# SeanSoraghan/Feature-Extractor

Hardware: AMD Instinct MI355X
Metric: frames/sec (1024-pt FFT, 10-feature bundle) (higher is better)
Workload: dtype f32

## Files before the change

### feature-extractor_amd/build.py

```python
import os
import shutil
import subprocess

HERE = os.path.dirname(os.path.abspath(__file__))
CSRC = os.path.join(HERE, "csrc")
LIB_DIR = os.path.join(HERE, "lib")
LIB_PATH = os.path.join(LIB_DIR, "libfx_hip.so")
HOST_SOURCES = ["fx_capi.cpp", "fx_plan.cpp", "fx_stream.cpp", "fx_comm.cpp", "fx_osc_sender.cpp"]
SOURCES = ["fx_kernels.hip", "fx_offline.hip", "fx_reblock.hip", "fx_osc.hip", "fx_taps.hip", "fx_interleave.hip", "fx_events.hip", "fx_tracks.hip", "fx_osc_table.hip", "fx_osc_bundle.hip"] + HOST_SOURCES
UNITS = [("fx_kernels.hip", "fx_kernels_small.o", ["-DFX_PART=1", "-mllvm", "-amdgpu-use-amdgpu-trackers=1"]),
         ("fx_kernels.hip", "fx_kernels_large.o", ["-DFX_PART=2"]),
         ("fx_kernels.hip", "fx_kernels_hop.o", ["-DFX_PART=3"]),
         ("fx_offline.hip", "fx_offline.o", []),
         ("fx_reblock.hip", "fx_reblock.o", []),
         ("fx_osc.hip", "fx_osc.o", []),
         ("fx_taps.hip", "fx_taps.o", []),
         ("fx_interleave.hip", "fx_interleave.o", []),
         ("fx_events.hip", "fx_events.o", []),
         ("fx_tracks.hip", "fx_tracks.o", []),
         ("fx_osc_table.hip", "fx_osc_table.o", []),
         ("fx_osc_bundle.hip", "fx_osc_bundle.o", [])] + [(s, s.replace(".cpp", ".o"), []) for s in HOST_SOURCES]
HEADERS = ["fx_kernels.h", "fx_context.h", "fx_plan.h", "fx_osc_words.h", "fx_wave.hip.h", "fx_lane_exchange.h", "fx_fft.hip.h", "fx_blocks.hip.h", "fx_frame_kernel.hip.h", "fx_pair_kernel.hip.h", "fx_tail_kernels.hip.h", "fx_hop_kernel.hip.h",
           os.path.join("..", "..", "include", "fx.h")]

HIPCC_FLAGS = ["--offload-arch=gfx950", "-O3", "-std=c++17", "-fPIC", "-ffp-contract=off",
               "-fno-fast-math", "-mllvm", "-disable-machine-licm", "-Wall", "-Wno-unused-function",
               "-Xclang", "-target-feature", "-Xclang", "-load-store-opt"]
HIPCC_FLAGS += os.environ.get("FX_EXTRA_HIPCC_FLAGS", "").split()


def flags_for_window(window):
    return HIPCC_FLAGS + (UNITS[0][2][1:] if window <= 1024 else [])


def _hipcc():
    exe = shutil.which("hipcc") or "/opt/rocm/bin/hipcc"
    if not os.path.exists(exe):
        raise RuntimeError("hipcc not found; cannot build libfx_hip.so")
    return exe


def _run(cmd):
    import sys
    proc = subprocess.run(cmd, stderr=subprocess.PIPE, text=True)
    for line in proc.stderr.splitlines():
        if "is not a recognized feature for this target" not in line:
            print(line, file=sys.stderr)
    if proc.returncode != 0:
        raise subprocess.CalledProcessError(proc.returncode, cmd)


FLAGS_STAMP = os.path.join(LIB_DIR, ".build.flags")


def _flags_stamp():
    return " ".join(HIPCC_FLAGS) + " | " + " ; ".join("%s:%s" % (o, " ".join(x)) for _, o, x in UNITS)


def needs_build():
    if not os.path.exists(LIB_PATH):
        return True
    try:
        if open(FLAGS_STAMP).read() != _flags_stamp():
            return True
    except OSError:
        return True
    t = os.path.getmtime(LIB_PATH)
    deps = [os.path.join(CSRC, s) for s in SOURCES + HEADERS] + [os.path.abspath(__file__)]
    return any(os.path.getmtime(d) > t for d in deps)


def build(force=False, verbose=False):
    if not force and not needs_build():
        return LIB_PATH
    import fcntl
    os.makedirs(LIB_DIR, exist_ok=True)
    with open(os.path.join(LIB_DIR, ".build.lock"), "w") as lock:
        fcntl.flock(lock, fcntl.LOCK_EX)
        try:
            if not force and not needs_build():
                return LIB_PATH
            tag = ".tmp%d" % os.getpid()
            objs = [os.path.join(LIB_DIR, objname) for _, objname, _ in UNITS]

            def compile_unit(unit):
                src, objname, extra = unit
                obj = os.path.join(LIB_DIR, objname)
                cmd = [_hipcc()] + HIPCC_FLAGS + extra + ["-x", "hip", "-c", os.path.join(CSRC, src), "-o", obj + tag]
                if verbose:
                    print(" ".join(cmd))
                _run(cmd)
                os.replace(obj + tag, obj)

            from concurrent.futures import ThreadPoolExecutor
            with ThreadPoolExecutor(max_workers=min(4, os.cpu_count() or 1)) as pool:
                list(pool.map(compile_unit, UNITS))
            cmd = [_hipcc(), "--offload-arch=gfx950", "-shared", "-fPIC", "-o", LIB_PATH + tag] + objs + ["-ldl", "-lpthread"]
            if verbose:
                print(" ".join(cmd))
            subprocess.check_call(cmd)
            os.replace(LIB_PATH + tag, LIB_PATH)
            with open(FLAGS_STAMP, "w") as f:
                f.write(_flags_stamp())
        finally:
            fcntl.flock(lock, fcntl.LOCK_UN)
    return LIB_PATH


if __name__ == "__main__":
    print(build(force=True, verbose=True))
```

### feature-extractor_amd/csrc/fx_fft.hip.h

```cpp


#include "fx_lane_exchange.h"

template <int N> struct Geo {
    static constexpr int M      = N / 2;
    static constexpr int P      = N / 64;
    static constexpr int U      = M / 64;
    static constexpr bool SPLIT = N >= 2048;
    static constexpr int RQ     = P > 16 ? P : 16;
    static constexpr int RIMG   = N + 4 * (N / RQ);
    static constexpr int BQ     = U >= 8 ? U : 0;
    static constexpr int BIMG   = M + (BQ ? 4 * (M / U) : 0);
    static constexpr int QSLOTS = N / 2 + (N == 2048 ? 8 * (N / 128) : 0);
    static constexpr int CSLOTS = SPLIT ? (cpad(N / 2 - 1) + 1 > QSLOTS ? cpad(N / 2 - 1) + 1 : QSLOTS) : cpad(N) + 2;
    static constexpr int CBUF_B = 8 * CSLOTS;
    static constexpr int RBUF_B = 4 * (SPLIT ? RIMG - 4 : RIMG + 4);
    static constexpr int HBUF_B = 4 * BIMG + 2 * M + 16;
    static constexpr int BUF_B0 = CBUF_B > RBUF_B ? (CBUF_B > HBUF_B ? CBUF_B : HBUF_B) : (RBUF_B > HBUF_B ? RBUF_B : HBUF_B);
    static constexpr int BUF_BYTES = (BUF_B0 > 4 * N ? BUF_B0 : 4 * N) + 15 & ~15;
    static constexpr int LOG2N  = (N == 256) ? 8 : (N == 512) ? 9 : (N == 1024) ? 10 : (N == 2048) ? 11 : 12;
    static constexpr int RA     = (N == 256) ? 4 : ((N == 512 || N == 2048) ? 8 : 16);
    static constexpr int LOG2RA = (RA == 4) ? 2 : (RA == 8) ? 3 : 4;
    static constexpr int ITEMS_A = N / RA;
    static constexpr int GA     = ITEMS_A / 64;
    static constexpr int IDIG   = (LOG2N - LOG2RA) / 2;
};

template <int N> __host__ __device__ constexpr int rimg(int n) { return n + 4 * (int) ((unsigned) n / (unsigned) Geo<N>::RQ); }
template <int N> __host__ __device__ constexpr int bimg(int b) { return Geo<N>::BQ ? b + 4 * (int) ((unsigned) b / (unsigned) (Geo<N>::BQ ? Geo<N>::BQ : 1)) : b; }
template <int N> __host__ __device__ constexpr int bimg_step(int c) { return Geo<N>::BQ ? c + 4 * (c / (Geo<N>::BQ ? Geo<N>::BQ : 1)) : c; }
template <int N> __host__ __device__ constexpr int rimg_step(int c) { return c + 4 * (c / Geo<N>::RQ); }
static_assert(64 % Geo<1024>::RQ == 0 && 64 % Geo<2048>::RQ == 0 && 64 % Geo<4096>::RQ == 0 && 64 % Geo<4096>::U == 0, "lane + 64*c splits");

template <int U> __device__ __forceinline__ void lds_load_block(const float* base, float (&out)[U])
{
    if (U % 4 == 0) {
#pragma unroll
        for (int j = 0; j < U; j += 4) {
            const f4 v = *reinterpret_cast<const f4*>(base + j);
            out[j] = v.x; out[j + 1] = v.y; out[j + 2] = v.z; out[j + 3] = v.w;
        }
    } else {
#pragma unroll
        for (int j = 0; j < U; j += 2) {
            const f2 v = *reinterpret_cast<const f2*>(base + j);
            out[j] = v.x; out[j + 1] = v.y;
        }
    }
}
template <int U> __device__ __forceinline__ void lds_store_block(float* base, const float (&in)[U])
{
    if (U % 4 == 0) {
#pragma unroll
        for (int j = 0; j < U; j += 4) *reinterpret_cast<f4*>(base + j) = f4{in[j], in[j + 1], in[j + 2], in[j + 3]};
    } else {
#pragma unroll
        for (int j = 0; j < U; j += 2) *reinterpret_cast<f2*>(base + j) = f2{in[j], in[j + 1]};
    }
}

template <bool INV> __device__ __forceinline__ f2 twmul(f2 a, f2 t)
{
    f2 p, q, r;
#ifdef FX_EXP_FMA_TWIDDLES
    if (INV) {
        asm("v_pk_mul_f32 %0, %1, %2 op_sel_hi:[0,1] neg_hi:[0,1]" : "=v"(p) : "v"(a), "v"(t));
        asm("v_pk_fma_f32 %0, %1, %2, %3 op_sel:[1,1,0] op_sel_hi:[1,0,1]" : "=v"(r) : "v"(a), "v"(t), "v"(p));
    } else {
        asm("v_pk_mul_f32 %0, %1, %2 op_sel_hi:[0,1]" : "=v"(p) : "v"(a), "v"(t));
        asm("v_pk_fma_f32 %0, %1, %2, %3 op_sel:[1,1,0] op_sel_hi:[1,0,1] neg_lo:[0,1,0]" : "=v"(r) : "v"(a), "v"(t), "v"(p));
    }
    (void) q;
    return r;
#else
    if (INV) {
        asm("v_pk_mul_f32 %0, %1, %2 op_sel_hi:[0,1] neg_hi:[0,1]" : "=v"(p) : "v"(a), "v"(t));
        asm("v_pk_mul_f32 %0, %1, %2 op_sel:[1,1] op_sel_hi:[1,0]" : "=v"(q) : "v"(a), "v"(t));
    } else {
        asm("v_pk_mul_f32 %0, %1, %2 op_sel_hi:[0,1]" : "=v"(p) : "v"(a), "v"(t));
        asm("v_pk_mul_f32 %0, %1, %2 op_sel:[1,1] op_sel_hi:[1,0] neg_lo:[0,1]" : "=v"(q) : "v"(a), "v"(t));
    }
    asm("v_pk_add_f32 %0, %1, %2" : "=v"(r) : "v"(p), "v"(q));
    return r;
#endif
}
template <bool INV> __device__ __forceinline__ f2 twmul_real(float r, f2 t)
{
    const f2 p = f2{r, r} * t;
    return INV ? f2{p.x, -p.y} : p;
}

template <bool NEG_HI> __device__ __forceinline__ f2 pk_add_rot(f2 a, f2 b)
{
    f2 r;
    if (NEG_HI) asm("v_pk_add_f32 %0, %1, %2 op_sel:[0,1] op_sel_hi:[1,0] neg_hi:[0,1]" : "=v"(r) : "v"(a), "v"(b));
    else        asm("v_pk_add_f32 %0, %1, %2 op_sel:[0,1] op_sel_hi:[1,0] neg_lo:[0,1]" : "=v"(r) : "v"(a), "v"(b));
    return r;
}

template <bool INV>
__device__ __forceinline__ void bfly4_core(f2& d0, f2& d1, f2& d2, f2& d3, f2 s0, f2 s1, f2 s2)
{
    const f2 s3 = s0 + s2;
    const f2 s4 = s0 - s2;
    const f2 s5 = d0 - s1;
    const f2 a = d0 + s1;
    d2 = a - s3;
    d0 = a + s3;
    if (INV) {
        d1 = pk_add_rot<false>(s5, s4);
        d3 = pk_add_rot<true>(s5, s4);
    } else {
        d1 = pk_add_rot<true>(s5, s4);
        d3 = pk_add_rot<false>(s5, s4);
    }
}
template <bool INV, bool ALL4, bool D0Y>
__device__ __forceinline__ void bfly4_re(f2& d0, f2& d1, f2& d2, f2& d3, f2 w1, f2 w2, f2 w3)
{
    const f2 s0 = twmul<INV>(d1, w1);
    const f2 s2 = twmul<INV>(d3, w3);
    float s1x, s1y = 0.0f;
    if (D0Y) { const f2 s1 = twmul<INV>(d2, w2); s1x = s1.x; s1y = s1.y; }
    else     s1x = INV ? (d2.x * w2.x) + (d2.y * w2.y) : (d2.x * w2.x) - (d2.y * w2.y);
    f2 t;
    asm("v_pk_add_f32 %0, %1, %2 neg_hi:[0,1]" : "=v"(t) : "v"(s0), "v"(s2));
    const float ax = d0.x + s1x, s5x = d0.x - s1x;
    const float y0 = D0Y ? (d0.y + s1y) + (s0.y + s2.y) : 0.0f;
    d0 = f2{ax + t.x, y0};
    d1 = f2{INV ? s5x - t.y : s5x + t.y, 0.0f};
    if (ALL4) {
        d2 = f2{ax - t.x, 0.0f};
        d3 = f2{INV ? s5x + t.y : s5x - t.y, 0.0f};
    }
}
template <bool INV>
__device__ __forceinline__ float bfly4_x0(f2 d0, f2 d1, f2 d2, f2 d3, f2 w1, f2 w2, f2 w3)
{
    const float s0x = INV ? (d1.x * w1.x) + (d1.y * w1.y) : (d1.x * w1.x) - (d1.y * w1.y);
    const float s1x = INV ? (d2.x * w2.x) + (d2.y * w2.y) : (d2.x * w2.x) - (d2.y * w2.y);
    const float s2x = INV ? (d3.x * w3.x) + (d3.y * w3.y) : (d3.x * w3.x) - (d3.y * w3.y);
    return (d0.x + s1x) + (s0x + s2x);
}
template <bool INV>
__device__ __forceinline__ void bfly4_real(float a0, float a1, float a2, float a3, f2& d0, f2& d1, f2& d2, f2& d3)
{
    const float s3 = a1 + a3, s4 = a1 - a3, s5 = a0 - a2, a = a0 + a2;
    d2 = f2{a - s3, 0.0f};
    d0 = f2{a + s3, 0.0f};
    d1 = f2{s5, INV ? s4 : -s4};
    d3 = f2{s5, INV ? -s4 : s4};
}

template <int N> struct Plan {
    static constexpr int R1 = 16;
    static constexpr int L1 = (N == 256) ? 4 : ((N == 512 || N == 2048) ? 8 : 16);
    static constexpr int R2 = (N >= 2048) ? 16 : 4;
    static constexpr int L2 = N / R2;
    static constexpr int OFF1 = 0;
    static constexpr int OFF2 = 15 * L1;
    static constexpr int OFFA = OFF2 + (R2 == 16 ? 15 : 3) * L2;
};

struct TwGlobal { const f2* table; bool quarter_turn; f2 at_quarter; };
template <int N> struct CompactTw {
    typedef Plan<N> PL;
    static constexpr int L2 = PL::L2;
    static constexpr int Q1_GAP = 16;
    static constexpr int OFF_S = 15 * PL::L1, OFF_Q1 = OFF_S + 3 * L2, OFF_GAP = OFF_Q1 + 2 * L2, OFF_R3 = OFF_Q1 + 4 * L2 + Q1_GAP, ENTRIES = OFF_R3 + 4 * L2;
    __host__ __device__ static constexpr int q1_pos(int j) { return (j >> 1) + ((j & 1) ? 2 * L2 + Q1_GAP : 0); }
    __host__ __device__ static constexpr int source(int e)
    {
        if (e < OFF_S)  return PL::OFF1 + e;
        if (e < OFF_Q1) return PL::OFF2 + (e - OFF_S);
        if (e < OFF_R3) {
            const int pos = e - OFF_Q1;
            if (pos >= 2 * L2 && pos < 2 * L2 + Q1_GAP) return -1;
            const int j = pos < 2 * L2 ? 2 * pos : 2 * (pos - 2 * L2 - Q1_GAP) + 1;
            return PL::OFF2 + (3 + 3 * (j / L2)) * L2 + j % L2;
        }
        return PL::OFF2 + (5 + 3 * ((e - OFF_R3) / L2)) * L2 + (e - OFF_R3) % L2;
    }
};
static_assert(CompactTw<4096>::ENTRIES == 3072 && CompactTw<4096>::OFF_S == 240 && CompactTw<4096>::q1_pos(1) == 528 && CompactTw<4096>::q1_pos(1022) == 511, "compact twiddle image");

enum { XK_POWER = 1, XK_SPECTRAL = 2, XK_RAW = 4, XK_INVERSE = 8 };
#define FX_XK_TEXT_(x) #x
#define FX_XK_TEXT(x) FX_XK_TEXT_(x)
constexpr unsigned lds_exchange_kinds(const char* text, unsigned shipped)
{
    if (text[0] < '0' || text[0] > '9') return shipped;
    unsigned v = 0;
    for (; *text >= '0' && *text <= '9'; text++) v = 10 * v + (unsigned) (*text - '0');
    return v;
}
constexpr unsigned LDS_EXCHANGE_KINDS = lds_exchange_kinds(FX_XK_TEXT(FX_EXP_LDS_EXCHANGE), 0u);
static_assert(LDS_EXCHANGE_KINDS <= 15u, "FX_EXP_LDS_EXCHANGE: a mask of the four transform kinds");

template <int N> struct RealExchange {
    static constexpr bool USE = N == 1024 || N == 4096;
    static constexpr int RA = Geo<N>::RA;
    static constexpr int SLOTS = RA == 16 ? 11 : 7;
    static constexpr int GROUP_PAD = RA == 16 ? 0 : 8;
    static constexpr unsigned long long SLOT_OF = RA == 16 ? 0x1a93487675439210ull
                                                           : 0x62543210ull;
    static constexpr unsigned TWIN = RA == 16 ? (1u << 3) | (1u << 7) | (1u << 11) | (1u << 12) | (1u << 15) : (1u << 6);
    __host__ __device__ static constexpr int stored(int q)
    {
        constexpr int s16[11] = {0, 1, 2, 4, 5, 6, 8, 9, 10, 13, 14};
        constexpr int s8[7] = {0, 1, 2, 3, 4, 5, 7};
        return RA == 16 ? s16[q < 11 ? q : 0] : s8[q < 7 ? q : 0];
    }
    __host__ __device__ static constexpr int row(int item) { return item * SLOTS + GROUP_PAD * (item / 16); }
};

template <int N, int R, int L0, int TWOFF, bool INV, bool FROM_REAL = false>
__device__ __forceinline__ void fft_pass(f2* cbuf, const f2* tw, int lane)
{
    constexpr int ITEMS = N / R;
    for (int it = lane; it < ITEMS; it += 64) {
        f2 e[R];
        const int k = it % L0;
        const int base = (it / L0) * (R * L0) + k;
        f2* img = cbuf + cpad(base);
        const f2* t1 = tw + TWOFF + k;
        if constexpr (FROM_REAL) {
            static_assert(R == 16 && L0 == 16 && ITEMS == 64, "the pass behind a 16-element real first pass");
            const int slot = (int) ((RealExchange<N>::SLOT_OF >> (4 * k)) & 15ull);
            const unsigned flip = ((RealExchange<N>::TWIN >> k) & 1u) << 31;
            const f2* src = cbuf + RealExchange<N>::row((it / L0) * 16) + slot;
#pragma unroll
            for (int i = 0; i < R; i++) {
                const f2 v = src[i * RealExchange<N>::SLOTS];
                e[i] = f2{v.x, __uint_as_float(__float_as_uint(v.y) ^ flip)};
            }
        } else {
#pragma unroll
            for (int i = 0; i < R; i++) e[i] = img[item_off(L0, i)];
        }
        {
            const f2 w1 = t1[0], w2 = t1[L0], w3 = t1[2 * L0];
#pragma unroll
            for (int g = 0; g < R / 4; g++)
                bfly4_core<INV>(e[4 * g], e[4 * g + 1], e[4 * g + 2], e[4 * g + 3],
                                twmul<INV>(e[4 * g + 1], w1), twmul<INV>(e[4 * g + 2], w2), twmul<INV>(e[4 * g + 3], w3));
        }
        if constexpr (R == 16) {
            const f2* t2 = t1 + 3 * L0;
#pragma unroll
            for (int jin = 0; jin < 4; jin++) {
                const f2 w1 = t2[(jin * 3 + 0) * L0], w2 = t2[(jin * 3 + 1) * L0], w3 = t2[(jin * 3 + 2) * L0];
                bfly4_core<INV>(e[jin], e[jin + 4], e[jin + 8], e[jin + 12],
                                twmul<INV>(e[jin + 4], w1), twmul<INV>(e[jin + 8], w2), twmul<INV>(e[jin + 12], w3));
            }
        }
#pragma unroll
        for (int i = 0; i < R; i++) img[item_off(L0, i)] = e[i];
    }
    wave_fence();
}

template <int DIGITS> __device__ __forceinline__ int rev4(int x)
{
    unsigned r = __builtin_bitreverse32((unsigned) x) >> (32 - 2 * DIGITS);
    r = ((r & 0x55555555u) << 1) | ((r >> 1) & 0x55555555u);
    return (int) r;
}

template <int N> __device__ __forceinline__ float bartlett_gain(int n)
{
    const float inc = 2.0f / N;
    return n < N / 2 ? (float) n * inc : 1.0f - (float) (n - N / 2) * inc;
}

template <int N> __device__ __forceinline__ int first_pass_index(int lane, int g, int j)
{
    typedef Geo<N> G;
    const int revj = (G::RA == 4) ? j : (G::RA == 8) ? ((j >> 1) + 4 * (j & 1)) : ((j >> 2) + 4 * (j & 3));
    return rev4<G::IDIG>(lane + 64 * g) + G::ITEMS_A * revj;
}

template <int N> __device__ __forceinline__ int first_pass_rbase(int lane, int g) { return rimg<N>(rev4<Geo<N>::IDIG>(lane + 64 * g)); }
template <int N> __host__ __device__ constexpr int first_pass_rstep(int j)
{
    return (Geo<N>::ITEMS_A + 4 * (Geo<N>::ITEMS_A / Geo<N>::RQ))
         * ((Geo<N>::RA == 4) ? j : (Geo<N>::RA == 8) ? ((j >> 1) + 4 * (j & 1)) : ((j >> 2) + 4 * (j & 3)));
}
static_assert(Geo<256>::ITEMS_A % Geo<256>::RQ == 0 && Geo<512>::ITEMS_A % Geo<512>::RQ == 0 && Geo<1024>::ITEMS_A % Geo<1024>::RQ == 0
              && Geo<2048>::ITEMS_A % Geo<2048>::RQ == 0 && Geo<4096>::ITEMS_A % Geo<4096>::RQ == 0, "the real image splits only at multiples of RQ");

template <int N, bool INV>
__device__ __forceinline__ void first_pass_item(const float* x, const f2 (&ta)[9], f2 (&e)[Geo<N>::RA])
{
    constexpr int R = Geo<N>::RA;
    if constexpr (R == 4) {
        bfly4_real<INV>(x[0], x[1], x[2], x[3], e[0], e[1], e[2], e[3]);
    } else if constexpr (R == 8) {
        float r[8];
#pragma unroll
        for (int h = 0; h < 4; h++) { r[2 * h] = x[2 * h] + x[2 * h + 1]; r[2 * h + 1] = x[2 * h] - x[2 * h + 1]; }
        bfly4_real<INV>(r[0], r[2], r[4], r[6], e[0], e[2], e[4], e[6]);
        e[1] = f2{r[1], 0.0f};
        bfly4_core<INV>(e[1], e[3], e[5], e[7], twmul_real<INV>(r[3], ta[0]), twmul_real<INV>(r[5], ta[1]), twmul_real<INV>(r[7], ta[2]));
    } else {
#pragma unroll
        for (int h = 0; h < 4; h++)
            bfly4_real<INV>(x[4 * h], x[4 * h + 1], x[4 * h + 2], x[4 * h + 3], e[4 * h], e[4 * h + 1], e[4 * h + 2], e[4 * h + 3]);
        {
            f2 o0, o1, o2, o3;
            bfly4_real<INV>(e[0].x, e[4].x, e[8].x, e[12].x, o0, o1, o2, o3);
            e[0] = o0; e[4] = o1; e[8] = o2; e[12] = o3;
        }
        bfly4_core<INV>(e[1], e[5], e[9], e[13], twmul<INV>(e[5], ta[0]), twmul<INV>(e[9], ta[1]), twmul<INV>(e[13], ta[2]));
        bfly4_core<INV>(e[2], e[6], e[10], e[14], twmul_real<INV>(e[6].x, ta[3]), twmul_real<INV>(e[10].x, ta[4]), twmul_real<INV>(e[14].x, ta[5]));
        e[3] = f2{e[13].x, -e[13].y}; e[7] = f2{e[9].x, -e[9].y}; e[11] = f2{e[5].x, -e[5].y}; e[15] = f2{e[1].x, -e[1].y};
    }
}

template <int N, bool INV>
__device__ __forceinline__ void fft_first_pass(const float (&xin)[Geo<N>::P], f2* cbuf, const float (&ftw)[18], int lane)
{
    typedef Geo<N> G;
    constexpr int R = G::RA;
    f2 ta[9];
#pragma unroll
    for (int i = 0; i < 9; i++) ta[i] = f2{ftw[2 * i], ftw[2 * i + 1]};
#pragma unroll
    for (int g = 0; g < G::GA; g++) {
        f2 e[R];
        first_pass_item<N, INV>(&xin[g * R], ta, e);
        if constexpr (RealExchange<N>::USE) {
            static_assert(R == 16 && G::GA == 1, "one 16-element item per lane");
            f2* img = cbuf + RealExchange<N>::row(lane);
#pragma unroll
            for (int q = 0; q < RealExchange<N>::SLOTS; q++) img[q] = e[RealExchange<N>::stored(q)];
        } else {
            f2* img = cbuf + cpad((lane + 64 * g) * R);
#pragma unroll
            for (int i = 0; i < R; i++) img[i] = e[i];
        }
    }
    wave_fence();
}

template <int L0, bool INV>
__device__ __forceinline__ void item16_stages(f2 (&e)[16], const f2* t1)
{
    {
        const f2 w1 = t1[0], w2 = t1[L0], w3 = t1[2 * L0];
#pragma unroll
        for (int g = 0; g < 4; g++)
            bfly4_core<INV>(e[4 * g], e[4 * g + 1], e[4 * g + 2], e[4 * g + 3],
                            twmul<INV>(e[4 * g + 1], w1), twmul<INV>(e[4 * g + 2], w2), twmul<INV>(e[4 * g + 3], w3));
    }
    const f2* t2 = t1 + 3 * L0;
#pragma unroll
    for (int jin = 0; jin < 4; jin++) {
        const f2 w1 = t2[(jin * 3 + 0) * L0], w2 = t2[(jin * 3 + 1) * L0], w3 = t2[(jin * 3 + 2) * L0];
        bfly4_core<INV>(e[jin], e[jin + 4], e[jin + 8], e[jin + 12],
                        twmul<INV>(e[jin + 4], w1), twmul<INV>(e[jin + 8], w2), twmul<INV>(e[jin + 12], w3));
    }
}

template <bool INV>
__device__ __forceinline__ void item16_stages_r(f2 (&e)[16], const f2 (&w)[15])
{
#pragma unroll
    for (int g = 0; g < 4; g++)
        bfly4_core<INV>(e[4 * g], e[4 * g + 1], e[4 * g + 2], e[4 * g + 3],
                        twmul<INV>(e[4 * g + 1], w[0]), twmul<INV>(e[4 * g + 2], w[1]), twmul<INV>(e[4 * g + 3], w[2]));
#pragma unroll
    for (int jin = 0; jin < 4; jin++)
        bfly4_core<INV>(e[jin], e[jin + 4], e[jin + 8], e[jin + 12],
                        twmul<INV>(e[jin + 4], w[3 + 3 * jin]), twmul<INV>(e[jin + 8], w[4 + 3 * jin]), twmul<INV>(e[jin + 12], w[5 + 3 * jin]));
}

template <int N, bool INV>
__device__ __forceinline__ void fft_second_pass_regs(const f2* cbuf, const f2* tw, int lane, f2 (&e)[16])
{
    typedef Plan<N> PL;
    static_assert(LaneExchange<N>::AVAILABLE && RealExchange<N>::USE && PL::R1 == 16 && PL::L1 == 16 && N / 16 == 64, "one second-pass item per lane");
    const int k = lane % 16;
    const int slot = (int) ((RealExchange<N>::SLOT_OF >> (4 * k)) & 15ull);
    const unsigned flip = ((RealExchange<N>::TWIN >> k) & 1u) << 31;
    const f2* src = cbuf + RealExchange<N>::row((lane / 16) * 16) + slot;
#pragma unroll
    for (int i = 0; i < 16; i++) {
        const f2 v = src[i * RealExchange<N>::SLOTS];
        e[i] = f2{v.x, __uint_as_float(__float_as_uint(v.y) ^ flip)};
    }
    wave_fence();
    item16_stages<PL::L1, INV>(e, tw + PL::OFF1 + k);
}

template <bool HALVES> __device__ __forceinline__ void lane_swap(f2& a, f2& b)
{
    const auto x = HALVES ? __builtin_amdgcn_permlane32_swap(__float_as_uint(a.x), __float_as_uint(b.x), false, false)
                          : __builtin_amdgcn_permlane16_swap(__float_as_uint(a.x), __float_as_uint(b.x), false, false);
    const auto y = HALVES ? __builtin_amdgcn_permlane32_swap(__float_as_uint(a.y), __float_as_uint(b.y), false, false)
                          : __builtin_amdgcn_permlane16_swap(__float_as_uint(a.y), __float_as_uint(b.y), false, false);
    a = f2{__uint_as_float(x[0]), __uint_as_float(y[0])};
    b = f2{__uint_as_float(x[1]), __uint_as_float(y[1])};
}
template <int N> __device__ __forceinline__ void second_exchange_regs(f2 (&e)[16])
{
    typedef LaneExchange<N> LX;
#pragma unroll
    for (int j = 0; j < LX::SWAPS; j++) lane_swap<true>(e[LX::swap(0, j).first], e[LX::swap(0, j).second]);
#pragma unroll
    for (int j = 0; j < LX::SWAPS; j++) lane_swap<false>(e[LX::swap(1, j).first], e[LX::swap(1, j).second]);
}

enum { OUT_RE_LOW = 1,
       OUT_RE_LOW_MAXABS = 2,
       OUT_POWER = 3,
       OUT_LAG = 4 };

template <int N, bool INV, int OUT> constexpr bool lane_exchange_used()
{
    return LaneExchange<N>::AVAILABLE && !(LDS_EXCHANGE_KINDS & (INV || OUT == OUT_LAG ? XK_INVERSE : OUT == OUT_POWER ? XK_POWER : OUT == OUT_RE_LOW_MAXABS ? XK_SPECTRAL : XK_RAW));
}

template <bool INV, int OUT, typename W>
__device__ __forceinline__ void item16_last(f2 (&e)[16], W w, bool first_item)
{
    constexpr bool ALL4 = !(OUT == OUT_RE_LOW || OUT == OUT_RE_LOW_MAXABS);
#pragma unroll
    for (int g = 0; g < 4; g++)
        bfly4_core<INV>(e[4 * g], e[4 * g + 1], e[4 * g + 2], e[4 * g + 3],
                        twmul<INV>(e[4 * g + 1], w(0)), twmul<INV>(e[4 * g + 2], w(1)), twmul<INV>(e[4 * g + 3], w(2)));
#pragma unroll
    for (int jin = 0; jin < 4; jin++) {
        const f2 w1 = w(3 + 3 * jin), w2 = w(4 + 3 * jin), w3 = w(5 + 3 * jin);
        if (OUT == OUT_RE_LOW_MAXABS)
            bfly4_re<INV, ALL4, true>(e[jin], e[jin + 4], e[jin + 8], e[jin + 12], w1, w2, w3);
        else if (OUT == OUT_LAG && jin == 0 && first_item)
            bfly4_re<INV, ALL4, true>(e[jin], e[jin + 4], e[jin + 8], e[jin + 12], w1, w2, w3);
        else
            bfly4_re<INV, ALL4, false>(e[jin], e[jin + 4], e[jin + 8], e[jin + 12], w1, w2, w3);
    }
}

template <int N> struct TwRegs {
    static constexpr bool USE = N == 2048;
    static constexpr bool USE_C = USE;
    static constexpr int GB = USE_C ? (N / 16) / 64 : 1;
    f2 b[15];
    f2 c[GB][15];
    __device__ __forceinline__ void load(const f2* tw, int lane)
    {
        typedef Plan<N> PL;
        const f2* t1 = tw + PL::OFF1 + lane % PL::L1;
#pragma unroll
        for (int i = 0; i < 15; i++) b[i] = t1[i * PL::L1];
#pragma unroll
        for (int g = 0; g < (USE_C ? GB : 0); g++) {
            const f2* t2 = tw + PL::OFF2 + lane + 64 * g;
#pragma unroll
            for (int i = 0; i < 15; i++) c[g][i] = t2[i * PL::L2];
        }
    }
};

template <int N> __host__ __device__ constexpr int qpad(int q) { return N == 2048 ? q + 8 * (q >> 6) : q; }
static_assert(qpad<2048>(1023) < Geo<2048>::CSLOTS && qpad<4096>(2047) < Geo<4096>::CSLOTS, "half image fits the wave buffer");

template <int N, bool INV, int OUT>
__device__ __forceinline__ float fft_last_pass_consume(f2 (&e)[(N / Plan<N>::R2) / 64][Plan<N>::R2], f2* cbuf, const f2* tw, int lane, float scale, float* regs_out)
{
    typedef Plan<N> PL;
    constexpr int R = PL::R2, L0 = PL::L2, GI = (N / R) / 64, TWOFF = PL::OFF2;
    float* fbuf = reinterpret_cast<float*>(cbuf);
    float aux = 0.0f;
#pragma unroll
    for (int g = 0; g < GI; g++) {
        const int k = lane + 64 * g;
        const f2* t1 = tw + TWOFF + k;
        if constexpr (R == 16) {
            item16_stages<L0, INV>(e[g], t1);
        } else {
            const f2 w1 = t1[0], w2 = t1[L0], w3 = t1[2 * L0];
            constexpr bool ALL4 = !(OUT == OUT_RE_LOW || OUT == OUT_RE_LOW_MAXABS);
            if (OUT == OUT_RE_LOW_MAXABS || (OUT == OUT_LAG && g == 0)) bfly4_re<INV, ALL4, true>(e[g][0], e[g][1], e[g][2], e[g][3], w1, w2, w3);
            else bfly4_re<INV, ALL4, false>(e[g][0], e[g][1], e[g][2], e[g][3], w1, w2, w3);
        }
#pragma unroll
        for (int i = 0; i < R; i++) {
            const int bin = k + L0 * i;
            if (OUT == OUT_RE_LOW || OUT == OUT_RE_LOW_MAXABS) {
                if (i < R / 2) fbuf[bimg<N>(lane) + bimg_step<N>(64 * g + L0 * i)] = e[g][i].x;
                if (OUT == OUT_RE_LOW_MAXABS && i < R / 4) aux = fmaxf(aux, fmaxf(fabsf(e[g][i].x), fabsf(e[g][i].y)));
            } else if (OUT == OUT_POWER) {
                if constexpr (Geo<N>::GA == 1) {
                    constexpr int RA = Geo<N>::RA;
                    const int m = g + (L0 / 64) * i;
                    const int j = (RA == 4) ? m : (RA == 8) ? (2 * (m & 3) + (m >> 2)) : (4 * (m & 3) + (m >> 2));
                    regs_out[j] = __int_as_float(__builtin_amdgcn_ds_bpermute(
                        rev4<Geo<N>::IDIG>(lane) << 2, __float_as_int(e[g][i].x * e[g][i].x)));
                } else {
                    fbuf[rimg<N>(lane) + rimg_step<N>(64 * g + L0 * i)] = e[g][i].x * e[g][i].x;
                }
            } else {
                const float d = e[g][i].x * scale;
                regs_out[g + (L0 / 64) * i] = d * d * (float) bin;
            }
        }
        if (OUT == OUT_LAG && g == 0) { const float d = e[0][0].y * scale; aux = d * d * (float) N; }
    }
    wave_fence();
    return aux;
}

template <int N, bool INV, int OUT>
__device__ __forceinline__ float fft_last_pass_fused(f2* cbuf, const f2* tw, int lane, float scale, float* regs_out)
{
    typedef Plan<N> PL;
    constexpr int R = PL::R2, L0 = PL::L2, GI = (N / R) / 64;
    f2 e[GI][R];
#pragma unroll
    for (int g = 0; g < GI; g++) {
        const f2* img = cbuf + cpad(lane + 64 * g);
#pragma unroll
        for (int i = 0; i < R; i++) e[g][i] = img[item_off(L0, i)];
    }
    wave_fence();
    return fft_last_pass_consume<N, INV, OUT>(e, cbuf, tw, lane, scale, regs_out);
}

template <int N, bool INV, int OUT>
__device__ __forceinline__ float fft_last_passes_lanes(f2* cbuf, const f2* tw, int lane, float scale, float* regs_out)
{
    typedef LaneExchange<N> LX;
    f2 s[16];
    fft_second_pass_regs<N, INV>(cbuf, tw, lane, s);
    second_exchange_regs<N>(s);
    f2 e[4][4];
#pragma unroll
    for (int g = 0; g < 4; g++)
#pragma unroll
        for (int i = 0; i < 4; i++) e[g][i] = s[LX::register_of(g, i)];
    return fft_last_pass_consume<N, INV, OUT>(e, cbuf, tw, lane, scale, regs_out);
}

template <int N, int OUT>
__device__ __forceinline__ void last_item_reduce(const f2 (&e)[16], int k, float scale, float (&res)[16], float& aux)
{
#pragma unroll
    for (int i = 0; i < 16; i++) {
        if (OUT == OUT_RE_LOW || OUT == OUT_RE_LOW_MAXABS) {
            if (i < 8) res[i] = e[i].x;
            if (OUT == OUT_RE_LOW_MAXABS && i < 4) aux = fmaxf(aux, fmaxf(fabsf(e[i].x), fabsf(e[i].y)));
        } else if (OUT == OUT_POWER) {
            res[i] = e[i].x * e[i].x;
        } else {
            const float d = e[i].x * scale;
            res[i] = d * d * (float) (k + (N / 16) * i);
        }
    }
}

template <int N> struct LazyLag {
    static_assert(N == 1024, "four last-pass butterflies per lane, one 64-sample block per butterfly's output 0");
    typedef Plan<N> PL;
    static constexpr int L0 = PL::L2;
    f2 e[4][4];
    const f2* t1;
    float scale;
    int lane;
    __device__ __forceinline__ void load(const float (&xin)[Geo<N>::P], f2* cbuf, const f2* tw, const float (&ftw)[18], int lane_, float scale_)
    {
        fft_first_pass<N, true>(xin, cbuf, ftw, lane_);
        lane = lane_;
        scale = scale_;
        t1 = tw + PL::OFF2 + lane;
        if constexpr (lane_exchange_used<N, true, OUT_LAG>()) {
            f2 s[16];
            fft_second_pass_regs<N, true>(cbuf, tw, lane, s);
            second_exchange_regs<N>(s);
#pragma unroll
            for (int g = 0; g < 4; g++)
#pragma unroll
                for (int i = 0; i < 4; i++) e[g][i] = s[LaneExchange<N>::register_of(g, i)];
        } else {
            fft_pass<N, PL::R1, PL::L1, PL::OFF1, true, RealExchange<N>::USE>(cbuf, tw, lane_);
#pragma unroll
            for (int g = 0; g < 4; g++) {
                const f2* img = cbuf + cpad(lane + 64 * g);
#pragma unroll
                for (int i = 0; i < 4; i++) e[g][i] = img[item_off(L0, i)];
            }
            wave_fence();
        }
    }
    __device__ __forceinline__ float head(int g) const
    {
        const f2* t = t1 + 64 * g;
        const float d = bfly4_x0<true>(e[g][0], e[g][1], e[g][2], e[g][3], t[0], t[L0], t[2 * L0]) * scale;
        return d * d * (float) (lane + 64 * g);
    }
    __device__ __forceinline__ float rest(float (&vreg)[Geo<N>::P])
    {
        float v_end = 0.0f;
#pragma unroll
        for (int g = 0; g < 4; g++) {
            const f2* t = t1 + 64 * g;
            if (g == 0) bfly4_re<true, true, true>(e[g][0], e[g][1], e[g][2], e[g][3], t[0], t[L0], t[2 * L0]);
            else        bfly4_re<true, true, false>(e[g][0], e[g][1], e[g][2], e[g][3], t[0], t[L0], t[2 * L0]);
#pragma unroll
            for (int i = 0; i < 4; i++) {
                const float d = e[g][i].x * scale;
                vreg[g + 4 * i] = d * d * (float) (lane + 64 * g + L0 * i);
            }
            if (g == 0) { const float d = e[0][0].y * scale; v_end = d * d * (float) N; }
        }
        return v_end;
    }
};

template <int N, bool INV, int OUT, bool CTW = false>
__device__ __forceinline__ float fft_split(const float (&xin)[Geo<N>::P], f2* cbuf, const f2* tw, const float (&ftw)[18],
                                           int lane, float scale, float* regs_out, const TwRegs<N>* twr, TwGlobal tg = TwGlobal{nullptr, false, f2{0.0f, 0.0f}})
{
    typedef Geo<N> G;
    typedef Plan<N> PL;
    constexpr int RA = G::RA, GA = G::GA, L1 = PL::L1, L2 = PL::L2, GB = (N / 16) / 64, HB = GB / 2;
    static_assert(PL::R1 == 16 && PL::R2 == 16 && GA == 4 && GB >= 2 && GB % 2 == 0, "split plan: three passes, even item counts");
    lane = opaque<N>(lane);
    f2 ta[9];
#pragma unroll
    for (int i = 0; i < 9; i++) ta[i] = f2{ftw[2 * i], ftw[2 * i + 1]};
    f2 eb[GB][16];
#pragma unroll
    for (int h = 0; h < 2; h++) {
#pragma unroll
        for (int gl = 0; gl < GA / 2; gl++) {
            f2 e[RA];
            first_pass_item<N, INV>(&xin[(h * (GA / 2) + gl) * RA], ta, e);
            if constexpr (RealExchange<N>::USE) {
                static_assert(RA == L1, "the next pass's stride is the item's length: its lanes read ONE element index each");
                f2* img = cbuf + RealExchange<N>::row(lane + 64 * gl);
#pragma unroll
                for (int q = 0; q < RealExchange<N>::SLOTS; q++) img[q] = e[RealExchange<N>::stored(q)];
            } else {
                f2* img = cbuf + cpad((lane + 64 * gl) * RA);
#pragma unroll
                for (int i = 0; i < RA; i++) img[i] = e[i];
            }
        }
        wave_fence();
#pragma unroll
        for (int jl = 0; jl < HB; jl++) {
            const int it = lane + 64 * jl;
            if constexpr (RealExchange<N>::USE) {
                const int k = it % L1;
                const int slot = (int) ((RealExchange<N>::SLOT_OF >> (4 * k)) & 15ull);
                const unsigned flip = ((RealExchange<N>::TWIN >> k) & 1u) << 31;
                const f2* src = cbuf + RealExchange<N>::row((it / L1) * 16) + slot;
#pragma unroll
                for (int i = 0; i < 16; i++) {
                    const f2 v = src[i * RealExchange<N>::SLOTS];
                    eb[h * HB + jl][i] = f2{v.x, __uint_as_float(__float_as_uint(v.y) ^ flip)};
                }
            } else {
                const f2* img = cbuf + cpad((it / L1) * (16 * L1) + it % L1);
#pragma unroll
                for (int i = 0; i < 16; i++) eb[h * HB + jl][i] = img[item_off(L1, i)];
            }
        }
        wave_fence();
#pragma unroll
        for (int jl = 0; jl < HB; jl++) {
            const int it = lane + 64 * jl;
            if constexpr (TwRegs<N>::USE) item16_stages_r<INV>(eb[h * HB + jl], twr->b);
            else item16_stages<L1, INV>(eb[h * HB + jl], tw + PL::OFF1 + it % L1);
        }
    }
    static_assert(16 * L1 == L2, "a second-pass item spans exactly one row of the last pass");
    float res[GB][16];
    float aux = 0.0f;
#pragma unroll
    for (int h = 0; h < 2; h++) {
#pragma unroll
        for (int j = 0; j < GB; j++) {
            const int it = lane + 64 * j;
            f2* img = cbuf + qpad<N>((L2 / 2) * (it / L1)) + it % L1;
#pragma unroll
            for (int i = 0; i < 8; i++) img[L1 * i] = eb[j][8 * h + i];
        }
        wave_fence();
        f2 ec[HB][16];
#pragma unroll
        for (int gl = 0; gl < HB; gl++) {
            const f2* img = cbuf + (lane + 64 * gl);
#pragma unroll
            for (int i = 0; i < 16; i++) ec[gl][i] = img[qpad<N>((L2 / 2) * i)];
        }
        wave_fence();
#pragma unroll
        for (int gl = 0; gl < HB; gl++) {
            const int g = h * HB + gl, k = lane + 64 * g;
            if constexpr (TwRegs<N>::USE_C) { const f2 (&wr)[15] = twr->c[g]; item16_last<INV, OUT>(ec[gl], [&](int i) { return wr[i]; }, g == 0); }
            else if constexpr (CTW) {
                static_assert(!TwRegs<N>::USE, "compact image: twiddles from LDS");
                typedef CompactTw<N> CT;
                const f2* at_lane = tw + lane;
                const f2* at_half = tw + CT::q1_pos(lane);
                const f2* ts = at_lane + (CT::OFF_S + 64 * g);
                const f2* q1 = at_half + (CT::OFF_Q1 + 32 * g);
                const f2* q2 = at_lane + (CT::OFF_Q1 + 64 * g);
                const f2* r3 = at_lane + (CT::OFF_R3 + 64 * g);
                item16_last<INV, OUT>(ec[gl], [&](int i) -> f2 {
                    if (i < 3) return ts[i * L2];
                    const int jin = (i - 3) / 3, q = (i - 3) % 3 + 1;
                    if (q == 1) return q1[jin * (L2 / 2)];
                    if (q == 3) return r3[jin * L2];
                    if (jin < 2) return q2[jin * L2];
                    if (!tg.quarter_turn) return tg.table[PL::OFF2 + k + i * L2];
                    const f2 t = q2[(jin - 2) * L2];
                    if (jin == 2 && g == 0 && lane == 0) return tg.at_quarter;
                    return f2{t.y, -t.x};
                }, g == 0);
            }
            else { const f2* t2 = tw + PL::OFF2 + k; item16_last<INV, OUT>(ec[gl], [&](int i) { return t2[i * L2]; }, g == 0); }
            last_item_reduce<N, OUT>(ec[gl], k, scale, res[g], aux);
            if (OUT == OUT_LAG && g == 0) { const float d = ec[0][0].y * scale; aux = d * d * (float) N; }
        }
    }
    float* fbuf = reinterpret_cast<float*>(cbuf);
#pragma unroll
    for (int g = 0; g < GB; g++) {
#pragma unroll
        for (int i = 0; i < 16; i++) {
            if (OUT == OUT_RE_LOW || OUT == OUT_RE_LOW_MAXABS) { if (i < 8) fbuf[bimg<N>(lane) + bimg_step<N>(64 * g + L2 * i)] = res[g][i]; }
            else if (OUT == OUT_POWER) fbuf[rimg<N>(lane) + rimg_step<N>(64 * g + L2 * i)] = res[g][i];
            else regs_out[g + (L2 / 64) * i] = res[g][i];
        }
    }
    wave_fence();
    return aux;
}

template <int N, bool INV, int OUT, bool CTW = false>
__device__ __forceinline__ float fft_from_regs(const float (&xin)[Geo<N>::P], f2* cbuf, const f2* tw, const float (&ftw)[18],
                                               int lane, float scale = 0.0f, float* regs_out = nullptr, const TwRegs<N>* twr = nullptr,
                                               TwGlobal tg = TwGlobal{nullptr, false, f2{0.0f, 0.0f}})
{
    typedef Plan<N> PL;
    static_assert(!CTW || Geo<N>::SPLIT, "the compact twiddle image belongs to a split transform");
    if constexpr (Geo<N>::SPLIT) {
        return fft_split<N, INV, OUT, CTW>(xin, cbuf, tw, ftw, lane, scale, regs_out, twr, tg);
    } else {
        fft_first_pass<N, INV>(xin, cbuf, ftw, lane);
        if constexpr (lane_exchange_used<N, INV, OUT>()) {
            return fft_last_passes_lanes<N, INV, OUT>(cbuf, tw, lane, scale, regs_out);
        } else {
            fft_pass<N, PL::R1, PL::L1, PL::OFF1, INV, RealExchange<N>::USE>(cbuf, tw, lane);
            return fft_last_pass_fused<N, INV, OUT>(cbuf, tw, lane, scale, regs_out);
        }
    }
}
```

### feature-extractor_amd/csrc/fx_frame_kernel.hip.h

```cpp
#define FX_OPQ(n, x) ((HOIST && ((n) == 15 || (n) == 0)) ? (x) : opaque<N>(x))
#ifdef FX_EXP_STOP_AT
#define FX_STOP(k, ...) if (FX_EXP_STOP_AT == (k)) { __VA_ARGS__; }
#else
#define FX_STOP(k, ...)
#endif
#define FX_KEEP(v) asm volatile("" :: "v"(v))

__device__ __forceinline__ constexpr int sample_bytes(int fmt) { return fmt == FX_SAMPLE_F32 ? 4 : (fmt == FX_SAMPLE_S24 ? 3 : 2); }
__device__ __forceinline__ float from_left_justified(unsigned w) { return (float) (int) w * (1.0f / 2147483648.0f); }
template <int FMT, bool LAST_USE = false> __device__ __forceinline__ float widen_one(const void* at)
{
    if (LAST_USE && FMT == FX_SAMPLE_F32) return __builtin_nontemporal_load(static_cast<const float*>(at));
    if (LAST_USE && FMT == FX_SAMPLE_S16) return (float) (int) __builtin_nontemporal_load(static_cast<const short*>(at)) * (1.0f / 32768.0f);
    if (LAST_USE && FMT == FX_SAMPLE_F16) return __half2float(__ushort_as_half(__builtin_nontemporal_load(static_cast<const unsigned short*>(at))));
    if (FMT == FX_SAMPLE_F16) return __half2float(*static_cast<const __half*>(at));
    if (FMT == FX_SAMPLE_S16) return (float) (int) *static_cast<const short*>(at) * (1.0f / 32768.0f);
    if (FMT == FX_SAMPLE_S24) {
        const unsigned char* b = static_cast<const unsigned char*>(at);
        return from_left_justified(((unsigned) b[0] << 8) | ((unsigned) b[1] << 16) | ((unsigned) b[2] << 24));
    }
    return *static_cast<const float*>(at);
}
template <int FMT> __device__ __forceinline__ f4 widen_four(uint4 r)
{
    if (FMT == FX_SAMPLE_S24)
        return f4{from_left_justified(r.x << 8), from_left_justified((r.y << 16) | ((r.x >> 16) & 0xff00u)),
                  from_left_justified((r.z << 24) | ((r.y >> 8) & 0xffff00u)), from_left_justified(r.z & 0xffffff00u)};
    if (FMT == FX_SAMPLE_F16) {
        const float2 a = __half22float2(*reinterpret_cast<const __half2*>(&r.x));
        const float2 b = __half22float2(*reinterpret_cast<const __half2*>(&r.y));
        return f4{a.x, a.y, b.x, b.y};
    }
    if (FMT == FX_SAMPLE_S16) {
        const f4 v = f4{(float) ((int) (r.x << 16) >> 16), (float) ((int) r.x >> 16), (float) ((int) (r.y << 16) >> 16), (float) ((int) r.y >> 16)};
        return v * (1.0f / 32768.0f);
    }
    return f4{__uint_as_float(r.x), __uint_as_float(r.y), __uint_as_float(r.z), __uint_as_float(r.w)};
}
template <int FMT> __device__ __forceinline__ uint4 fetch_four(const void* src, int i)
{
    if (FMT == FX_SAMPLE_F32) return *reinterpret_cast<const uint4*>(static_cast<const float*>(src) + i);
    if (FMT == FX_SAMPLE_S24) {
        const uint3 v = *reinterpret_cast<const uint3*>(static_cast<const unsigned char*>(src) + 3 * i);
        return uint4{v.x, v.y, v.z, 0u};
    }
    const uint2 v = *reinterpret_cast<const uint2*>(static_cast<const unsigned short*>(src) + i);
    return uint4{v.x, v.y, 0u, 0u};
}
#define FX_FORMATS(fa, fb, CALL) do {                                                                                              \
        if ((fb) == FX_SAMPLE_F16)      { if ((fa) == FX_SAMPLE_F16) { constexpr int FA = FX_SAMPLE_F16, FB = FX_SAMPLE_F16; CALL; }   \
                                          else                       { constexpr int FA = FX_SAMPLE_F32, FB = FX_SAMPLE_F16; CALL; } } \
        else if ((fb) == FX_SAMPLE_S16) { if ((fa) == FX_SAMPLE_S16) { constexpr int FA = FX_SAMPLE_S16, FB = FX_SAMPLE_S16; CALL; }   \
                                          else                       { constexpr int FA = FX_SAMPLE_F32, FB = FX_SAMPLE_S16; CALL; } } \
        else if ((fb) == FX_SAMPLE_S24) { if ((fa) == FX_SAMPLE_S24) { constexpr int FA = FX_SAMPLE_S24, FB = FX_SAMPLE_S24; CALL; }   \
                                          else                       { constexpr int FA = FX_SAMPLE_F32, FB = FX_SAMPLE_S24; CALL; } } \
        else                            { constexpr int FA = FX_SAMPLE_F32, FB = FX_SAMPLE_F32; CALL; }                                \
    } while (0)

template <int N, int HALF>
__device__ __forceinline__ void load_half(const void* src, int sample_format, float gain, bool apply_gain,
                                          float* rbuf, int dst_off, float* tail_out, int lane)
{
    for (int i = lane * 4; i < HALF; i += 256) {
        f4 v;
        if (sample_format == FX_SAMPLE_F16)      v = widen_four<FX_SAMPLE_F16>(fetch_four<FX_SAMPLE_F16>(src, i));
        else if (sample_format == FX_SAMPLE_S16) v = widen_four<FX_SAMPLE_S16>(fetch_four<FX_SAMPLE_S16>(src, i));
        else if (sample_format == FX_SAMPLE_S24) v = widen_four<FX_SAMPLE_S24>(fetch_four<FX_SAMPLE_S24>(src, i));
        else                                     v = widen_four<FX_SAMPLE_F32>(fetch_four<FX_SAMPLE_F32>(src, i));
        if (apply_gain) v *= gain;
        *reinterpret_cast<f4*>(&rbuf[rimg<N>(dst_off + i)]) = v;
        if (tail_out) *reinterpret_cast<f4*>(tail_out + i) = v;
    }
}

template <int N, int FMT_A, int FMT_B, bool BLOCKS = false>
__device__ __forceinline__ double load_window(const void* src_a, const void* src_b, float gain_a, float gain_b,
                                              float* rbuf, float* tail_out, int lane, const BlockStream bs = BlockStream{}, const bool a_stream = false,
                                              const BlockStream bs_a = BlockStream{})
{
    double ssq = 0.0;
    constexpr int HALF = N / 2, QH = HALF / 256;
    uint4 ra[QH], rb[QH];
#pragma unroll
    for (int q = 0; q < QH; q++) {
        if (BLOCKS && a_stream) ra[q] = stream_four<sample_bytes(FMT_A)>(bs_a, 256 * q + 4 * lane);
        else                           ra[q] = fetch_four<FMT_A>(src_a, 256 * q + 4 * lane);
    }
#pragma unroll
    for (int q = 0; q < QH; q++) {
        if constexpr (BLOCKS) rb[q] = stream_four<sample_bytes(FMT_B)>(bs, 256 * q + 4 * lane);
        else                  rb[q] = fetch_four<FMT_B>(src_b, 256 * q + 4 * lane);
    }
#pragma unroll
    for (int q = 0; q < QH; q++) {
        const int i = 256 * q + 4 * lane;
        const f4 v = widen_four<FMT_A>(ra[q]) * gain_a;
        *reinterpret_cast<f4*>(&rbuf[rimg<N>(i)]) = v;
        if (Geo<N>::SPLIT) ssq += (double) (v.x * v.x) + (double) (v.y * v.y) + (double) (v.z * v.z) + (double) (v.w * v.w);
    }
#pragma unroll
    for (int q = 0; q < QH; q++) {
        const int i = 256 * q + 4 * lane;
        const f4 v = widen_four<FMT_B>(rb[q]) * gain_b;
        *reinterpret_cast<f4*>(&rbuf[rimg<N>(HALF + i)]) = v;
        if (tail_out) *reinterpret_cast<f4*>(tail_out + i) = v;
        if (Geo<N>::SPLIT) ssq += (double) (v.x * v.x) + (double) (v.y * v.y) + (double) (v.z * v.z) + (double) (v.w * v.w);
    }
    return ssq;
}

template <int N, int FMT_A, int FMT_B, bool LAST_USE = false, bool BLOCKS = false>
__device__ __forceinline__ void load_window_first_pass_order(const void* src_a, const void* src_b, float gain_a, float gain_b,
                                                             int lane, float (&x)[Geo<N>::P], const BlockStream bs = BlockStream{}, const bool a_stream = false,
                                                             const BlockStream bs_a = BlockStream{})
{
    typedef Geo<N> G;
    static_assert(G::IDIG == 4 && G::GA == 4, "split sizes: 256 first-pass items, 4 per lane");
    const unsigned low = (unsigned) rev4<G::IDIG>(lane);
    const unsigned off_a = low * (unsigned) sample_bytes(FMT_A), off_b = low * (unsigned) sample_bytes(FMT_B);
#pragma unroll
    for (int g = 0; g < G::GA; g++) {
#pragma unroll
        for (int j = 0; j < G::RA; j++) {
            const int r = (G::RA == 4) ? j : (G::RA == 8) ? ((j >> 1) + 4 * (j & 1)) : ((j >> 2) + 4 * (j & 3));
            const bool second = r >= G::RA / 2;
            const int k = g + G::ITEMS_A * (second ? r - G::RA / 2 : r);
            if constexpr (BLOCKS) {
                if (second) {
                    x[g * G::RA + j] = widen_one<FMT_B, LAST_USE>(stream_sample<sample_bytes(FMT_B)>(bs, (int) low + k));
                    continue;
                }
                if (a_stream) {
                    x[g * G::RA + j] = widen_one<FMT_A, LAST_USE>(stream_sample<sample_bytes(FMT_A)>(bs_a, (int) low + k));
                    continue;
                }
            }
            const char* at = static_cast<const char*>(second ? src_b : src_a) + (second ? off_b : off_a) + k * sample_bytes(second ? FMT_B : FMT_A);
            x[g * G::RA + j] = second ? widen_one<FMT_B, LAST_USE>(at) : widen_one<FMT_A, LAST_USE>(at);
        }
    }
    if (gain_a != 1.0f || gain_b != 1.0f) {
#pragma unroll
        for (int g = 0; g < G::GA; g++)
#pragma unroll
            for (int j = 0; j < G::RA; j++) {
                const int r = (G::RA == 4) ? j : (G::RA == 8) ? ((j >> 1) + 4 * (j & 1)) : ((j >> 2) + 4 * (j & 3));
                x[g * G::RA + j] *= (r >= G::RA / 2) ? gain_b : gain_a;
            }
    }
}

struct FlatProd { double mant; int exp; };

__device__ __forceinline__ FlatProd fp_mul(FlatProd a, double m)
{
    const double p = a.mant * m;
    FlatProd r;
    r.exp = a.exp + __builtin_amdgcn_frexp_exp(p);
    r.mant = __builtin_amdgcn_frexp_mant(p);
    return r;
}
__device__ __forceinline__ FlatProd fp_mul2(FlatProd a, FlatProd b)
{
    const double p = a.mant * b.mant;
    FlatProd r;
    r.exp = a.exp + b.exp + __builtin_amdgcn_frexp_exp(p);
    r.mant = __builtin_amdgcn_frexp_mant(p);
    return r;
}

template <int N> struct LagSearch {
    float lag, run, carry, best;
    int first, best_i;
    bool done;
    __device__ __forceinline__ void begin()
    {
        lag = -1.0f;
        run = 0.0f;
        carry = 0.0f;
        first = 0x7fffffff;
        done = false;
        best = 100.0f; best_i = 0x7fffffff;
    }
    __device__ __forceinline__ void block(int lane, int blk, float v)
    {
        const int s_ = 64 * blk + lane;
        const float addend = (s_ == 0) ? 0.0f : v;
        float sm = lane == 0 ? run + addend : addend;
#pragma unroll
        for (int k = 1; k < 64; k++)
            asm volatile("s_nop 1\n\tv_add_f32_dpp %0, %0, %1 wave_shr:1 row_mask:0xf bank_mask:0xf" : "+v"(sm) : "v"(addend));
        run = __int_as_float(__builtin_amdgcn_readlane(__float_as_int(sm), 63));
        const float c_ = (sm != 0.0f) ? v / sm : 0.0f;
        const float p_ = shift_up1(c_, carry);
        carry = __int_as_float(__builtin_amdgcn_readlane(__float_as_int(c_), 63));
        if (s_ >= 2 && c_ < best) { best = c_; best_i = s_; }
        if (first == 0x7fffffff) {
            const unsigned long long hit = wave_ballot(c_ < 0.01f) & (blk == 0 ? ~3ull : ~0ull);
            if (hit) first = 64 * blk + (int) __builtin_ctzll(hit);
        }
        if (first != 0x7fffffff) {
            const int k0 = first + 1 - 64 * blk;
            const unsigned long long st = wave_ballot(!(c_ < p_)) & (k0 <= 0 ? ~0ull : (k0 >= 64 ? 0ull : ~0ull << k0));
            if (st) {
                const int src = (int) __builtin_ctzll(st);
                const float pc = lane_get(p_, src), cc = lane_get(c_, src);
                const int sstar = 64 * blk + src;
                lag = (pc <= cc) ? (float) (sstar - 1) : (float) sstar;
                done = true;
            }
        }
    }
    __device__ __forceinline__ float finish(int lane, float v_end)
    {
        if (!done) {
            if (first != 0x7fffffff) {
                float cn = 0.0f;
                if (lane == 0) { run += v_end; cn = (run != 0.0f) ? v_end / run : 0.0f; }
                cn = __int_as_float(__builtin_amdgcn_readfirstlane(__float_as_int(cn)));
                lag = (carry <= cn) ? (float) (N - 1) : (float) N;
            } else {
#pragma unroll
                for (int o = 32; o > 0; o >>= 1) {
                    const float ov = __shfl_xor(best, o, 64);
                    const int oi = __shfl_xor(best_i, o, 64);
                    if (ov < best || (ov == best && oi < best_i)) { best = ov; best_i = oi; }
                }
                lag = best_i == 0x7fffffff ? -1.0f : (float) best_i;
            }
        }
        return lag;
    }
};

template <int N> struct Occ {
    static constexpr int WAVES_PER_SIMD = N <= 512 ? 8 : (N <= 1024 ? 4 : 2);
    static constexpr int MAX_THREADS = 512;
};

template <int N> struct FrameLds {
    static constexpr bool WIDE = N == 4096;
    static constexpr int TW_ENTRIES = WIDE ? CompactTw<N>::ENTRIES : N;
    static constexpr int WIDE_TURN_ENTRY = WIDE ? CompactTw<N>::OFF_GAP : 0;
    __host__ __device__ static constexpr int prev_floats(bool direct) { return (direct || WIDE) ? 0 : Geo<N>::BIMG + (Geo<N>::BQ ? 0 : 4); }
    __host__ __device__ static constexpr size_t bytes(int ch, int k, bool direct)
    {
        return sizeof(f2) * TW_ENTRIES + (size_t) ch * sizeof(float) * prev_floats(direct) + (size_t) ch * k * Geo<N>::BUF_BYTES;
    }
};
static_assert(FrameLds<4096>::bytes(1, 8, false) <= 160 * 1024 && FrameLds<4096>::bytes(8, 1, true) <= 160 * 1024, "eight 4096-point wavefronts per CU");

template <int N, bool DIRECT = false, bool HOIST = false, bool WIDE = false, bool BLOCKS = false> struct FrameWave {
    typedef Geo<N> G;
    static constexpr int M = G::M, P = G::P, U = G::U, HALF = N / 2;

    const FrameParams& p;
    const f2* tw;
    __device__ __forceinline__ TwGlobal tw_global() const { return TwGlobal{reinterpret_cast<const f2*>(p.tw), p.tw_quarter_turn != 0, f2{p.tw_at_quarter[0], p.tw_at_quarter[1]}}; }
    const TwRegs<N>* twr;
    float* prev;
    int*   turn;
    f2*    cbuf;
    float* rbuf;
    FramePart* fpl;
    double nyquist, rnyq, frpb;
    float  scale;
    int    c, T, t;

    struct HarmonicSpectrum { float hre[U]; float left2, left1, right1; double sum, max; };

    struct Sources { const void* a; const void* b; float gain_a, gain_b; int fmt_a, fmt_b; BlockStream bs, bs_a; bool a_stream; };
    __device__ __forceinline__ Sources sources() const
    {
        const size_t esz = (size_t) sample_bytes(p.sample_format);
        const unsigned char* in = static_cast<const unsigned char*>(p.in);
        Sources s;
        s.fmt_a = s.fmt_b = p.sample_format;
        if constexpr (BLOCKS) {
            const BlockStream base{p.blk_carry_in + (size_t) c * (size_t) p.blk_carry_row_bytes, in + (size_t) c * (size_t) p.blk_in_row_bytes,
                                   p.blk_carry_bytes, p.blk_in_row_bytes};
            const long long hop_bytes = (long long) HALF * (long long) esz;
            const int tt = DIRECT ? 0 : __builtin_amdgcn_readfirstlane(t);
            s.bs = stream_from(base, (long long) (p.blk_hop0 + tt) * hop_bytes);
            s.b = nullptr; s.gain_b = p.gain;
            s.a_stream = !DIRECT && tt > 0;
            if (DIRECT || tt == 0) { s.a = p.tail_in + (size_t) c * HALF; s.fmt_a = FX_SAMPLE_F32; s.gain_a = 1.0f; s.bs_a = s.bs; }
            else        { s.a = nullptr; s.gain_a = p.gain; s.bs_a = stream_from(base, (long long) (p.blk_hop0 + tt - 1) * hop_bytes); }
            return s;
        }
        s.a_stream = false;
        if (p.hop_mode) {
            s.gain_a = s.gain_b = p.gain;
            const size_t row = (size_t) c * (size_t) (p.in_hop_stride ? p.in_hop_stride : T) + (size_t) p.in_hop0;
            s.b = in + (row + t) * HALF * esz;
            if (t == 0) { s.a = p.tail_in + (size_t) c * HALF; s.fmt_a = FX_SAMPLE_F32; s.gain_a = 1.0f; }
            else        s.a = in + (row + (t - 1)) * HALF * esz;
        } else {
            s.gain_a = s.gain_b = 1.0f;
            s.a = in + ((size_t) c * T + t) * N * esz;
            s.b = static_cast<const unsigned char*>(s.a) + HALF * esz;
        }
        return s;
    }

    template <bool LAST_USE = false>
    __device__ __forceinline__ void load_raw(int lane, float (&x)[P]) const
    {
        asm volatile("" ::: "memory");
        const Sources s = sources();
        FX_FORMATS(s.fmt_a, s.fmt_b, (load_window_first_pass_order<N, FA, FB, LAST_USE, BLOCKS>(s.a, s.b, s.gain_a, s.gain_b, lane, x, s.bs, s.a_stream, s.bs_a)));
    }

    __device__ __forceinline__ double load_frame(int lane) const
    {
FX_MARK("load");
        double ssq = 0.0;
        {
            float* tail_dst = (t == T - 1) ? p.tail_out + (size_t) c * HALF : nullptr;
            const Sources sr = sources();
            const void* src_a = sr.a; const void* src_b = sr.b;
            const float gain_a = sr.gain_a, gain_b = sr.gain_b;
            if constexpr (N >= 512) {
                FX_FORMATS(sr.fmt_a, sr.fmt_b, (ssq = load_window<N, FA, FB, BLOCKS>(src_a, src_b, gain_a, gain_b, rbuf, tail_dst, lane, sr.bs, sr.a_stream, sr.bs_a)));
            } else {
                load_half<N, HALF>(src_a, sr.fmt_a, gain_a, gain_a != 1.0f, rbuf, 0, nullptr, lane);
                load_half<N, HALF>(src_b, sr.fmt_b, gain_b, gain_b != 1.0f, rbuf, HALF, tail_dst, lane);
            }
            wave_fence();
        }
        return ssq;
    }

    __device__ __forceinline__ double sum_squares(int lane, float (&xr)[P]) const
    {
FX_MARK("rms");
#pragma unroll
        for (int g = 0; g < G::GA; g++)
#pragma unroll
            for (int j = 0; j < G::RA; j++) xr[g * G::RA + j] = (rbuf + first_pass_rbase<N>(lane, g))[first_pass_rstep<N>(j)];
        wave_fence();
        double s = 0.0;
#pragma unroll
        for (int i = 0; i < P; i++) s += (double) (xr[i] * xr[i]);
        s = wave_sum(s);
        if (lane == 0) fpl->sum_sq = s;
        return s;
    }

    static __device__ __forceinline__ float exact_log_rms(double sum_sq)
    {
        const float rms = (float) sqrt(sum_sq / (double) N);
        return (float) log10((double) (rms * 9.0f + 1.0f));
    }

    __device__ __forceinline__ float gate_threshold(double sum_sq, const float (&re)[U]) const
    {
#ifdef FX_EXP_WIDE_BAND
        const float rel = 0.5f, abs_ = 0.5f;
#else
        const float rel = 1e-4f, abs_ = 4e-6f;
#endif
        const float rms_a = __builtin_amdgcn_sqrtf((float) (sum_sq * (1.0 / (double) N)));
        const float log_a = __builtin_amdgcn_logf(rms_a * 9.0f + 1.0f) * 0.30103f;
        const float eps_lo = 0.01f * (log_a * (1.0f - rel) - abs_);
        const float eps_hi = 0.01f * (log_a * (1.0f + rel) + abs_);
        const float t_lo = __builtin_amdgcn_sqrtf(fmaxf(eps_lo, 0.0f)) * (1.0f - 1e-6f);
        const float t_hi = __builtin_amdgcn_sqrtf(eps_hi) * (1.0f + 1e-6f);
        bool inside = false;
#pragma unroll
        for (int j = 0; j < U; j++) inside |= (fabsf(re[j]) > t_lo) && !(fabsf(re[j]) > t_hi);
        if (!wave_any(inside)) return t_hi;
        const double eps = 0.01 * (double) exact_log_rms(sum_sq);
        float t = (float) sqrt(eps);
        const float up = __uint_as_float(__float_as_uint(t) + 1u);
        if ((double) t * (double) t > eps) t = __uint_as_float(__float_as_uint(t) - 1u);
        else if ((double) up * (double) up <= eps) t = up;
        return t;
    }

    __device__ __forceinline__ void flatness_local(const float (&re)[U], float tg, FlatProd& loc, int& emin, int& emax) const
    {
        loc = FlatProd{0.5, 1};
        emin = 1; emax = 1;
#pragma unroll
        for (int j = 0; j < U; j++) {
            const double v = (double) re[j];
            const double mag = v * v;
            if (fabsf(re[j]) > tg) {
                loc = fp_mul(loc, mag);
                emin = loc.exp < emin ? loc.exp : emin;
                emax = loc.exp > emax ? loc.exp : emax;
            }
        }
    }
    __device__ __forceinline__ double flatness_product(int lane, const float (&re)[U], float tg, FlatProd loc, int emin, int emax) const
    {
FX_MARK("flatprod");
        FlatProd inc = loc;
#define FX_FP_STEP(CTRL, ROW_MASK) { FlatProd nb; nb.mant = dpp_d<CTRL, ROW_MASK>(0.5, inc.mant); nb.exp = dpp_i<CTRL, ROW_MASK>(1, inc.exp); inc = fp_mul2(nb, inc); }
        FX_FP_STEP(DPP_ROW_SHR1, 0xF)
        FX_FP_STEP(DPP_ROW_SHR2, 0xF)
        FX_FP_STEP(DPP_ROW_SHR4, 0xF)
        FX_FP_STEP(DPP_ROW_SHR8, 0xF)
        FX_FP_STEP(DPP_BCAST15, 0xA)
        FX_FP_STEP(DPP_BCAST31, 0xC)
#undef FX_FP_STEP
        FlatProd exc;
        exc.mant = shift_up1(inc.mant, 0.5);
        exc.exp = shift_up1(inc.exp, 1);
        const unsigned long long risky_lanes = wave_ballot(exc.exp + emax >= 1025) | wave_ballot(exc.exp + emin - 1 <= -1022);
        if (risky_lanes == 0)
            return ldexp(bcast63(inc.mant), __builtin_amdgcn_readlane(inc.exp, 63));
        const int owner = (int) __builtin_ctzll(risky_lanes);
        double pr = ldexp(lane_get(exc.mant, owner), lane_get(exc.exp, owner));
        double factor[U];
#pragma unroll
        for (int j = 0; j < U; j++) {
            const double v = (double) re[j];
            const double mag = v * v;
            factor[j] = fabsf(re[j]) > tg ? mag : 1.0;
        }
        for (int l = owner; l < 64; l++) {
            double mine = pr;
#pragma unroll
            for (int j = 0; j < U; j++) mine *= factor[j];
            pr = lane_get(mine, l);
            if (pr == 0.0 || pr == __builtin_huge_val()) break;
        }
        return pr;
    }

    __device__ __forceinline__ void spectral(int lane, const float (&xr)[P], double sum_sq) const
    {
        float spec_aux = 0.0f;
FX_MARK("spec_fft");
        lane = FX_OPQ(0, lane);
        {
            float xw[P];
#pragma unroll
            for (int g = 0; g < G::GA; g++) {
                const float base = (float) rev4<G::IDIG>(lane + 64 * g) * (2.0f / N);
                const float nbase = 1.0f - base;
#pragma unroll
                for (int j = 0; j < G::RA; j++) {
                    const int r = (G::RA == 4) ? j : (G::RA == 8) ? ((j >> 1) + 4 * (j & 1)) : ((j >> 2) + 4 * (j & 3));
                    const float gain = r < G::RA / 2 ? base + (float) r * (2.0f / G::RA)
                                                     : nbase - (float) (r - G::RA / 2) * (2.0f / G::RA);
                    xw[g * G::RA + j] = xr[g * G::RA + j] * gain;
                }
            }
            spec_aux = fft_from_regs<N, false, OUT_RE_LOW_MAXABS, WIDE>(xw, cbuf, tw, p.first_tw, lane, 0.0f, nullptr, twr, tw_global());
        }
        FX_STOP(6, FX_KEEP(spec_aux); return);
FX_MARK("spec_sums");
        {
            float re[U];
            float maxabs = spec_aux;
            lds_load_block<U>(reinterpret_cast<const float*>(cbuf) + bimg<N>(U * lane), re);
            const float tg = gate_threshold(sum_sq, re);
            double Ts = 0.0, Vs = 0.0, Ws = 0.0, t_after = 0.0;
            double flat_sum = 0.0;
            float max_re = 0.0f;
            int cnt = 0;
            constexpr int LQ = (M / 5) / U, LR = (M / 5) % U;
#pragma unroll
            for (int j = U - 1; j >= 0; j--) {
                const double v = (double) re[j];
                const double mag = v * v;
                Ts += mag;
                if (j >= 1) { Vs += Ts; Ws += Vs; }
                if (j == LR + 1) t_after = Ts;
                const bool gate = fabsf(re[j]) > tg;
                cnt += __builtin_popcountll(wave_ballot(gate));
                if (gate) flat_sum += mag;
                max_re = fmaxf(max_re, fabsf(re[j]));
            }
            FlatProd floc; int femin, femax;
            if constexpr (!G::SPLIT) flatness_local(re, tg, floc, femin, femax);
            const double ul = (double) (U * lane);
            double mag_sum = Ts;
            double b1 = ul * Ts + Vs;
            double b2 = (ul * ul) * Ts + ((ul + ul) * Vs + ((Ws + Ws) - Vs));
            double lhr = lane < LQ ? Ts : (lane == LQ ? Ts - t_after : 0.0);
            wave_sum4(lane, mag_sum, b1, b2, lhr);
            max_re = wave_maxf(max_re);
            const double max_mag = (double) max_re * (double) max_re;
            maxabs = wave_maxf(maxabs);
            const bool accepted = mag_sum > 0.05;

            FX_STOP(7, FX_KEEP(mag_sum); FX_KEEP(b1); FX_KEEP(b2); FX_KEEP(lhr); FX_KEEP(max_mag); FX_KEEP(maxabs); FX_KEEP(flat_sum); FX_KEEP(cnt);
                       FX_KEEP(floc.mant); FX_KEEP(floc.exp); FX_KEEP(femin); FX_KEEP(femax); return);
FX_MARK("flux");
            double flux = 0.0;
            {
                float pvf[U];
                if constexpr (DIRECT) {
                    float* state = p.prev_re + (size_t) c * M + U * lane;
                    lds_load_block<U>(state, pvf);
                    if (accepted) lds_store_block<U>(state, re);
                } else if constexpr (WIDE) {
                    while (__hip_atomic_load(turn, __ATOMIC_ACQUIRE, __HIP_MEMORY_SCOPE_WORKGROUP) != t)
                        __builtin_amdgcn_s_sleep(1);
                    float* state = p.prev_re + (size_t) c * M + U * lane;
                    lds_load_block<U>(state, pvf);
                    if (accepted) lds_store_block<U>(state, re);
                    __builtin_amdgcn_fence(__ATOMIC_RELEASE, "workgroup");
                    if (lane == 0) __hip_atomic_store(turn, t + 1, __ATOMIC_RELEASE, __HIP_MEMORY_SCOPE_WORKGROUP);
                } else {
                    while (__hip_atomic_load(turn, __ATOMIC_ACQUIRE, __HIP_MEMORY_SCOPE_WORKGROUP) != t)
                        __builtin_amdgcn_s_sleep(1);
                    lds_load_block<U>(prev + bimg<N>(U * lane), pvf);
                    if (accepted) lds_store_block<U>(prev + bimg<N>(U * lane), re);
                    __builtin_amdgcn_fence(__ATOMIC_RELEASE, "workgroup");
                    if (lane == 0) __hip_atomic_store(turn, t + 1, __ATOMIC_RELEASE, __HIP_MEMORY_SCOPE_WORKGROUP);
                }
#pragma unroll
                for (int j = 0; j < U; j++) {
                    const double pv = (double) pvf[j];
                    const double v = (double) re[j];
                    const double diff = v * v - pv * pv;
                    flux += fmax(diff, 0.0);
                }
            }
            FX_STOP(8, FX_KEEP(mag_sum); FX_KEEP(b1); FX_KEEP(b2); FX_KEEP(lhr); FX_KEEP(max_mag); FX_KEEP(maxabs); FX_KEEP(flat_sum); FX_KEEP(cnt);
                       FX_KEEP(floc.mant); FX_KEEP(floc.exp); FX_KEEP(femin); FX_KEEP(femax); FX_KEEP(flux); return);
            lane = FX_OPQ(1, lane);
            if constexpr (G::SPLIT) flatness_local(re, tg, floc, femin, femax);
            const double prod = flatness_product(lane, re, tg, floc, femin, femax);
            FX_STOP(9, FX_KEEP(mag_sum); FX_KEEP(b1); FX_KEEP(b2); FX_KEEP(lhr); FX_KEEP(max_mag); FX_KEEP(maxabs); FX_KEEP(flat_sum); FX_KEEP(cnt);
                       FX_KEEP(prod); FX_KEEP(flux); return);

FX_MARK("spec_pass2");
            {
                const double mu = mag_sum * (1.0 / (double) M);
                double vsum = 0.0;
#pragma unroll
                for (int j = 0; j < U; j++) {
                    const double v = (double) re[j];
                    const double dv = __builtin_fma(v, v, -mu);
                    vsum = __builtin_fma(dv, dv, vsum);
                }
                const double wm = b1 + 0.5 * mag_sum, s2b0 = (b2 + b1 + 0.25 * mag_sum) * mag_sum, ww = wm * wm;
                const bool refine = accepted && (!(s2b0 - ww > 1e-9 * ww) || !(s2b0 < __builtin_huge_val()));
                double direct = 0.0;
                if (refine) {
                    const float centroid = (float) ((frpb * wm) / mag_sum);
                    const double cn = (double) centroid * rnyq;
#pragma unroll
                    for (int j = 0; j < U; j++) {
                        const double v = (double) re[j];
                        const double d = ((double) (U * lane + j) * frpb + (frpb / 2.0)) * rnyq - cn;
                        direct += (d * d) * (v * v);
                    }
                }
                wave_sum4(lane, flux, vsum, flat_sum, direct);
                if (lane == 0) { fpl->var = direct; fpl->refined = refine ? 1 : 0; fpl->vsum = vsum; }
            }
            double max_e = (double) maxabs;
            if (max_mag > max_e) max_e = max_mag;
            if (lane == 0) {
                fpl->mag_sum = mag_sum; fpl->lhr = lhr; fpl->flux = flux; fpl->flat_sum = flat_sum; fpl->prod = prod;
                fpl->max_e = max_e; fpl->b1 = b1; fpl->b2 = b2; fpl->cnt = (float) cnt;
            }
        }
        wave_fence();
    }

    __device__ __forceinline__ void harmonic_spectrum(int lane, const float (&xr)[P], HarmonicSpectrum& hs) const
    {
        float (&hre)[U] = hs.hre;
        float &h_left2 = hs.left2, &h_left1 = hs.left1, &h_right1 = hs.right1;
        double &h_sum = hs.sum, &h_max = hs.max;
        h_sum = 0.0;
        float h_max_re = 0.0f;
FX_MARK("harm1");
        lane = FX_OPQ(2, lane);
        fft_from_regs<N, false, OUT_RE_LOW, WIDE>(xr, cbuf, tw, p.first_tw, lane, 0.0f, nullptr, twr, tw_global());
        {
            const int b0 = U * lane;
            const float* relin = reinterpret_cast<const float*>(cbuf);
            lds_load_block<U>(relin + bimg<N>(b0), hre);
            h_left2  = b0 >= 2 ? fabsf(relin[bimg<N>(b0 - 2)]) : 0.0f;
            h_left1  = b0 >= 1 ? fabsf(relin[bimg<N>(b0 - 1)]) : 0.0f;
            h_right1 = b0 + U < M ? fabsf(relin[bimg<N>(b0 + U)]) : 0.0f;
#pragma unroll
            for (int j = 0; j < U; j++) {
                const double v = (double) hre[j];
                h_sum += v * v;
                h_max_re = fmaxf(h_max_re, fabsf(hre[j]));
            }
            h_sum = wave_sum(h_sum);
            h_max_re = wave_maxf(h_max_re);
            h_max = (double) h_max_re * (double) h_max_re;
        }
        wave_fence();
    }

    template <int K> static __device__ __forceinline__ void scaled_pairs(float a, const float* in, float* out)
    {
#pragma unroll
        for (int i = 0; i < K; i += 2) {
            const f2 t = f2{in[i], in[i + 1]} * a;
            out[i] = t.x; out[i + 1] = t.y;
            asm volatile("" : "+v"(out[i]), "+v"(out[i + 1]));
        }
    }
    __device__ __forceinline__ void lowpass_window(int lane) const
    {
FX_MARK("lpf");
                constexpr int KW = 16;
        const float a = p.lpf_a, b = p.lpf_b;
        float x[P];
#pragma unroll
        for (int i = 0; i < P; i += 4) {
            const f4 v = *reinterpret_cast<const f4*>(&rbuf[rimg<N>(P * lane + i)]);
            x[i] = v.x; x[i + 1] = v.y; x[i + 2] = v.z; x[i + 3] = v.w;
        }
        float yin = 0.0f;
        {
            const int first = P * lane;
#pragma unroll
            for (int q = 0; q < KW / 4; q++) {
                const int n0 = first - KW + 4 * q;
                if (n0 >= 0) {
                    const f4 v = *reinterpret_cast<const f4*>(&rbuf[rimg<N>(n0)]);
                    const float w[4] = {v.x, v.y, v.z, v.w};
                    float aw[4];
                    scaled_pairs<4>(a, w, aw);
#pragma unroll
                    for (int e = 0; e < 4; e++)
                        yin = (n0 + e == 0 || (q == 0 && e == 0)) ? w[e] : aw[e] + (b * yin);
                }
            }
        }
        wave_fence();
        float y[P];
        float ylast;
        constexpr int AXN = G::SPLIT ? 4 : P;
        float ax[AXN];
        {
            float yy = yin;
#pragma unroll
            for (int i = 0; i < P; i += AXN) {
                scaled_pairs<AXN>(a, &x[i], ax);
#pragma unroll
                for (int e = 0; e < AXN; e++) {
                    yy = (lane == 0 && i + e == 0) ? x[0] : ax[e] + (b * yy);
                    y[i + e] = yy;
                }
            }
            ylast = yy;
        }
        for (int iter = 0; iter < 64; iter++) {
            const float pe = shift_up1(ylast, 0.0f);
            const unsigned long long bad_lanes = wave_ballot(__float_as_uint(pe) != __float_as_uint(yin)) & ~1ull;
            if (!bad_lanes) break;
            if ((bad_lanes >> lane) & 1) {
                yin = pe;
                float yy = yin;
#pragma unroll
                for (int i = 0; i < P; i++) { yy = (AXN == P ? ax[i % AXN] : a * x[i]) + (b * yy); y[i] = yy; }
                ylast = yy;
            }
        }
        lane = FX_OPQ(3, lane);
        const float w0 = bartlett_gain<N>(P * lane);
        const float wstep = lane < 32 ? (2.0f / N) : -(2.0f / N);
#pragma unroll
        for (int i = 0; i < P; i += 4) {
            f4 v;
            v.x = y[i]     * __builtin_fmaf(wstep, (float) i, w0);
            v.y = y[i + 1] * __builtin_fmaf(wstep, (float) (i + 1), w0);
            v.z = y[i + 2] * __builtin_fmaf(wstep, (float) (i + 2), w0);
            v.w = y[i + 3] * __builtin_fmaf(wstep, (float) (i + 3), w0);
            *reinterpret_cast<f4*>(&rbuf[rimg<N>(P * lane + i)]) = v;
        }
        wave_fence();
    }

    template <bool LAZY>
    __device__ __forceinline__ float lag_search(int lane, float (&vreg)[P], float v_end, LazyLag<LAZY ? N : 1024>* lz) const
    {
FX_MARK("scan");
        lane = FX_OPQ(4, lane);
        LagSearch<N> ls;
        ls.begin();
        ls.block(lane, 0, vreg[0]);
        if (!ls.done && P > 1) ls.block(lane, 1, vreg[1]);
        if (!ls.done && P > 2) {
            float* vbuf = rbuf;
            if constexpr (LAZY) {
                vbuf[64 * 2 + lane] = lz->head(2);
                vbuf[64 * 3 + lane] = lz->head(3);
                wave_fence();
                for (int blk = 2; blk < P && !ls.done; blk++) {
                    if (blk == 4) {
                        v_end = lz->rest(vreg);
#pragma unroll
                        for (int m = 4; m < P; m++) vbuf[64 * m + lane] = vreg[m];
                        wave_fence();
                    }
                    ls.block(lane, blk, vbuf[64 * blk + lane]);
                }
            } else {
#pragma unroll
                for (int m = 2; m < P; m++) vbuf[64 * m + lane] = vreg[m];
                wave_fence();
                for (int blk = 2; blk < P && !ls.done; blk++) ls.block(lane, blk, vbuf[64 * blk + lane]);
            }
        }
        return ls.finish(lane, v_end);
    }

    __device__ __forceinline__ double pitch(int lane) const
    {
        lowpass_window(FX_OPQ(5, lane));
        FX_STOP(2, return 1.0);
FX_MARK("pitch_fft");
        lane = FX_OPQ(6, lane);
        float xf[P];
#pragma unroll
        for (int g = 0; g < G::GA; g++)
#pragma unroll
            for (int j = 0; j < G::RA; j++) xf[g * G::RA + j] = (rbuf + first_pass_rbase<N>(lane, g))[first_pass_rstep<N>(j)];
        wave_fence();
        float xp[P];
        fft_from_regs<N, false, OUT_POWER, WIDE>(xf, cbuf, tw, p.first_tw, lane, 0.0f, xp, twr, tw_global());
        FX_STOP(3, for (int j = 0; j < P; j++) FX_KEEP(xp[j]); return 1.0);
FX_MARK("power");
        lane = FX_OPQ(7, lane);
        if constexpr (G::GA == 1) {
#pragma unroll
            for (int j = 0; j < P; j++) xf[j] = xp[j];
        } else {
#pragma unroll
            for (int g = 0; g < G::GA; g++)
#pragma unroll
                for (int j = 0; j < G::RA; j++) xf[g * G::RA + j] = (rbuf + first_pass_rbase<N>(lane, g))[first_pass_rstep<N>(j)];
            wave_fence();
        }
FX_MARK("ifft");
        float vreg[P];
        float lag;
        if constexpr (N == 1024) {
            LazyLag<N> lz;
            lz.load(xf, cbuf, tw, p.first_tw, lane, scale);
            vreg[0] = lz.head(0);
            vreg[1] = lz.head(1);
            FX_STOP(4, FX_KEEP(vreg[0]); FX_KEEP(vreg[1]); return 1.0);
            lag = lag_search<true>(lane, vreg, 0.0f, &lz);
        } else
        {
            const float v_end = fft_from_regs<N, true, OUT_LAG, WIDE>(xf, cbuf, tw, p.first_tw, lane, scale, vreg, twr, tw_global());
            lag = lag_search<false>(lane, vreg, v_end, nullptr);
        }
        if (lane == 0) fpl->lag = lag;
        wave_fence();
        return (nyquist * 2.0) / (double) lag;
    }

    __device__ __forceinline__ void harmonic_tail(int lane, HarmonicSpectrum& hs, double f0) const
    {
        float (&hre)[U] = hs.hre;
        const float h_left2 = hs.left2, h_left1 = hs.left1, h_right1 = hs.right1;
        double &h_sum = hs.sum;
        const double h_max = hs.max;
FX_MARK("harm2");
        lane = FX_OPQ(8, lane);
        if (!(h_sum < 0.005)) {
            float* normed = reinterpret_cast<float*>(cbuf);
            unsigned short* peaks = reinterpret_cast<unsigned short*>(normed + G::BIMG);
            double mean_mag = h_sum / (double) M;
            {
                const float root_mean = __builtin_amdgcn_sqrtf((float) mean_mag);
                const float band = root_mean * 3e-6f;
                unsigned long long near = 0;
#pragma unroll
                for (int j = 0; j < U; j++) near |= wave_ballot(fabsf(fabsf(hre[j]) - root_mean) <= band);
                if (near) {
                    double run = 0.0;
                    for (int l = 0; l < 64; l++) {
                        double mine = run;
#pragma unroll
                        for (int j = 0; j < U; j++) { const double v = (double) hre[j]; mine += v * v; }
                        run = lane_get(mine, l);
                    }
                    h_sum = run;
                    mean_mag = h_sum / (double) M;
                }
            }
            bool pk[U];
            const double r_hmax = 1.0 / h_max;
            const double sum_normed = h_sum * r_hmax;
            int npk_lane = 0;
#pragma unroll
            for (int j = 0; j < U; j++) {
                const double v = (double) hre[j];
                const float me = fabsf(hre[j]);
                const float l2 = j >= 2 ? fabsf(hre[j >= 2 ? j - 2 : 0]) : (j == 1 ? h_left1 : h_left2);
                const float l1 = j >= 1 ? fabsf(hre[j >= 1 ? j - 1 : 0]) : h_left1;
                const float r1 = j + 1 < U ? fabsf(hre[j + 1 < U ? j + 1 : 0]) : h_right1;
                bool is_peak = v * v > mean_mag && !(l2 > me) && !(l1 > me);
                if (j == U - 2) is_peak = is_peak && (!(r1 > me) || lane == 63);
                else            is_peak = is_peak && !(r1 > me);
                pk[j] = is_peak;
                npk_lane += is_peak ? 1 : 0;
            }
            const int pre = wave_scan_incl_i(npk_lane);
            const int total_peaks = __builtin_amdgcn_readlane(pre, 63);
            {
                unsigned short* wp = peaks + (pre - npk_lane);
#pragma unroll
                for (int j = 0; j < U; j++)
                    if (pk[j]) { *wp = (unsigned short) (U * lane + j); wp++; }
            }
            wave_fence();

            const double fr = nyquist / (double) M;
            double probe = 0.0;
            int f0_bin;
            {
                const double freq = lane < 15 ? ldexp(f0, -(lane + 1)) : (lane < 18 ? f0 * (double) (lane - 14) : f0);
                int bin = (int) floor(freq / fr);
                f0_bin = __builtin_amdgcn_readlane(bin, 18);
                if (lane < 15) { if (bin == f0_bin) bin = -1; }
                else if (lane < 18) { if (bin >= M) bin = -1; }
                else bin = -1;
                if (bin >= 0 && bin < M) {
                    float mx = fabsf(normed[bimg<N>(bin)]);
                    const float a2 = bin >= 2 ? fabsf(normed[bimg<N>(bin >= 2 ? bin - 2 : 0)]) : mx;
                    const float a1 = bin >= 1 ? fabsf(normed[bimg<N>(bin >= 1 ? bin - 1 : 0)]) : mx;
                    const float b1 = bin + 1 < M ? fabsf(normed[bimg<N>(bin + 1 < M ? bin + 1 : 0)]) : mx;
                    float run = mx;
                    if (a2 > run) run = a2;
                    if (a1 > run) run = a1;
                    if (b1 > run) run = b1;
                    mx = run;
                    const double pm = (double) mx;
                    probe = (double) (float) ((pm * pm) * r_hmax);
                }
            }

            double inh = 0.0;
            const double r_hsum = 1.0 / h_sum;
            if (f0 > 0.0) {
                for (int i = lane; i < total_peaks; i += 64) {
                    const int bin = (int) peaks[i];
                    if (bin == f0_bin) continue;
                    double fs = (double) bin * fr;
                    if (fs == 0.0) fs = fr * 0.5;
                    const double fe = (double) (bin + 1) * fr;
                    const double rs  = (fs > f0 ? fs : f0) / (fs > f0 ? f0 : fs);
                    const double re_ = (fe > f0 ? fe : f0) / (fe > f0 ? f0 : fe);
                    if (floor(rs) != floor(re_)) continue;
                    const double r = rs < re_ ? rs : re_;
                    const double v = (double) normed[bimg<N>(bin)];
                    inh += (r - floor(r)) * ((v * v) * r_hsum);
                }
            }
            double score = probe;
            wave_sum2(lane, score, inh);
            if (lane == 0) { fpl->inh = inh; fpl->her_score = score; fpl->sum_normed = sum_normed; fpl->flags = 1; }
        }
        wave_fence();
    }
};

template <int N, bool SPEC, bool HARM, bool DIRECT, bool BLOCKS = false>
__device__ __forceinline__ void frame_kernel_body(const FrameParams& p_arg)
{
    static_assert(!BLOCKS || N >= 512, "the block-fed forms exist from 512 points on (load_window)");
    FrameParams p = p_arg;
    if (p.dyn) { p.gain = p.dyn->gain; p.nyquist = p.dyn->nyquist; }
    typedef Geo<N> G;
    constexpr int M = G::M, P = G::P;

    extern __shared__ __attribute__((aligned(16))) unsigned char smem[];
    constexpr bool WIDE = FrameLds<N>::WIDE;
    constexpr int PREV_FLOATS = FrameLds<N>::prev_floats(DIRECT);
    constexpr size_t WAVE_BYTES = G::BUF_BYTES;
    const int CH = p.ch_per_wg, K = p.waves_per_ch;
    f2*    tw    = reinterpret_cast<f2*>(smem);
    f2*    tw_lds = tw;
    float* prev0 = reinterpret_cast<float*>(tw_lds + FrameLds<N>::TW_ENTRIES);
    unsigned char* per_wave = reinterpret_cast<unsigned char*>(prev0 + (size_t) CH * PREV_FLOATS);

    const int wave = __builtin_amdgcn_readfirstlane((int) (threadIdx.x >> 6));
    const int lane0 = threadIdx.x & 63;
    const int chl = wave / K, slot = wave % K;
    const int T = p.T;
    int group = (int) blockIdx.x, chunk = 0;
    if (p.num_chunks > 1) {
        unsigned* ticket_s = reinterpret_cast<unsigned*>(per_wave);
        if (threadIdx.x == 0) *ticket_s = __hip_atomic_fetch_add(p.queue, 1u, __ATOMIC_RELAXED, __HIP_MEMORY_SCOPE_AGENT);
        __syncthreads();
        const unsigned ticket = *ticket_s, groups = gridDim.x / (unsigned) p.num_chunks;
        __syncthreads();
        chunk = (int) (ticket / groups);
        group = (int) (ticket % groups);
    }
    const int c = group * CH + chl;
    const bool live = c < p.C;
    if (live) p.gain = channel_gain(p, c);
    const int t_begin = p.num_chunks > 1 ? p_arg.chunk_begin[chunk] : 0;
    const int t_end = p.num_chunks > 1 ? p_arg.chunk_begin[chunk + 1] : T;

    float* prev = prev0 + (size_t) chl * PREV_FLOATS;
    int*   turn = WIDE ? reinterpret_cast<int*>(tw_lds + FrameLds<N>::WIDE_TURN_ENTRY) + 2 * chl : reinterpret_cast<int*>(G::BQ ? prev + G::U : prev + G::BIMG);
    f2*    cbuf = reinterpret_cast<f2*>(per_wave + WAVE_BYTES * wave);
    float* rbuf = reinterpret_cast<float*>(cbuf);

    if constexpr (WIDE) {
        typedef CompactTw<N> CT;
        const f2* image = reinterpret_cast<const f2*>(p.tw_image);
        for (int i = threadIdx.x; i < CT::ENTRIES; i += blockDim.x)
            if (i < CT::OFF_GAP || i >= CT::OFF_GAP + CT::Q1_GAP) tw_lds[i] = image[i];
    } else {
        for (int i = threadIdx.x; i < N; i += blockDim.x) tw_lds[i] = reinterpret_cast<const f2*>(p.tw)[i];
    }
    if (chunk > 0) {
        if (live && slot == 0 && lane0 == 0) {
            unsigned spins = 0;
            bool there;
            while (!(there = __hip_atomic_load(p.queue + 1 + c, __ATOMIC_RELAXED, __HIP_MEMORY_SCOPE_AGENT) >= (unsigned) chunk) && ++spins < p.spin_limit)
                __builtin_amdgcn_s_sleep(8);
            if (!there) __hip_atomic_store(p.err, 1u, __ATOMIC_RELAXED, __HIP_MEMORY_SCOPE_SYSTEM);
            __builtin_amdgcn_fence(__ATOMIC_ACQUIRE, "agent");
            asm volatile("s_waitcnt vmcnt(0)" ::: "memory");
        }
        __syncthreads();
    }
    if (live && !DIRECT) {
        if constexpr (!WIDE)
            for (int i = lane0 + 64 * slot; i < M; i += 64 * K) prev[bimg<N>(i)] = p.prev_re[(size_t) c * M + i];
        if (lane0 == 0 && slot == 0) { turn[0] = t_begin; turn[1] = t_begin; }
    }
    __syncthreads();

    TwRegs<N> twr;
    if constexpr (TwRegs<N>::USE) twr.load(tw, lane0);

    const double nyquist = p.nyquist;
    const double rnyq = 1.0 / nyquist;
    const double frpb = nyquist / (double) M;
    const float  scale = 1.0f / (float) N;

    constexpr bool CLAIM = (N == 4096) && !DIRECT;
    auto next_frame = [&](int t_now) -> int {
        if constexpr (!CLAIM) return t_now + K;
        int v = 0;
        if (lane0 == 0) v = __hip_atomic_fetch_add(turn + 1, 1, __ATOMIC_RELAXED, __HIP_MEMORY_SCOPE_WORKGROUP);
        return __builtin_amdgcn_readfirstlane(v);
    };
    for (int t = live ? (CLAIM ? next_frame(0) : t_begin + slot) : t_end; t < t_end; t = next_frame(t)) {
        constexpr bool HOIST = SPEC && !HARM && N == 1024;
        const int lane = FX_OPQ(15, lane0);
        FramePart* fpl = p.part + ((size_t) c * T + t);
        if (lane == 0) fpl->flags = 0;
        const FrameWave<N, DIRECT, HOIST, WIDE, BLOCKS> w{p, tw, &twr, prev, turn, cbuf, rbuf, fpl, nyquist, rnyq, frpb, scale, c, T, t};

        const double ssq_lane = w.load_frame(lane);
        float xr[P];
        double sum_sq;
        if constexpr (G::SPLIT) {
            sum_sq = wave_sum(ssq_lane);
            if (lane == 0) fpl->sum_sq = sum_sq;
        } else {
            sum_sq = w.sum_squares(lane, xr);
        }
        double f0 = 0.0;
        FX_STOP(1, FX_KEEP(sum_sq); FX_KEEP(xr[0]); continue);
        if constexpr (HARM) f0 = w.pitch(lane);
        FX_STOP(2, continue); FX_STOP(3, continue); FX_STOP(4, continue);
        FX_STOP(5, FX_KEEP(f0); continue);
        if constexpr (SPEC) {
            if constexpr (G::SPLIT) w.load_raw(lane, xr);
            w.spectral(lane, xr, sum_sq);
        }
        FX_STOP(6, continue); FX_STOP(7, continue); FX_STOP(8, continue); FX_STOP(9, continue); FX_STOP(10, continue);
        if constexpr (HARM) {
            typename FrameWave<N, DIRECT, HOIST, WIDE, BLOCKS>::HarmonicSpectrum hs;
            if constexpr (G::SPLIT) w.template load_raw<true>(lane, xr);
            w.harmonic_spectrum(lane, xr, hs);
            FX_STOP(11, FX_KEEP(hs.sum); FX_KEEP(hs.max); FX_KEEP(hs.left2); FX_KEEP(hs.left1); FX_KEEP(hs.right1); for (int j = 0; j < G::U; j++) FX_KEEP(hs.hre[j]); continue);
            w.harmonic_tail(lane, hs, f0);
        }
        if constexpr (BLOCKS)
            if (p.blk_keep_rest && t == T - 1)
                stream_keep_rest(w.sources().bs, (long long) (N / 2) * sample_bytes(p.sample_format), p.blk_carry_out + (size_t) c * (size_t) p.blk_carry_row_bytes, lane, 64);
    }

    if constexpr (DIRECT) return;
    __syncthreads();
    if constexpr (!WIDE)
        if (live)
            for (int i = lane0 + 64 * slot; i < M; i += 64 * K) p.prev_re[(size_t) c * M + i] = prev[bimg<N>(i)];
    if (chunk + 1 < p.num_chunks) {
        asm volatile("s_waitcnt vmcnt(0)" ::: "memory");
        __syncthreads();
        if (live && slot == 0 && lane0 == 0 && !(p.debug_flags & 1u)) {
            __builtin_amdgcn_fence(__ATOMIC_RELEASE, "agent");
            asm volatile("s_waitcnt vmcnt(0)" ::: "memory");
            __hip_atomic_store(p.queue + 1 + c, (unsigned) (chunk + 1), __ATOMIC_RELAXED, __HIP_MEMORY_SCOPE_AGENT);
        }
    }
}

template <int N, bool SPEC, bool HARM, bool DIRECT = false, bool BLOCKS = false>
__global__ void __launch_bounds__(Occ<N>::MAX_THREADS, Occ<N>::WAVES_PER_SIMD)
fx_frame_kernel(const FrameParams p_arg)
{
    frame_kernel_body<N, SPEC, HARM, DIRECT, BLOCKS>(p_arg);
}
```

Measured before the change: 197.0 million.

## Hoist per-lane LDS and twiddle addresses into a loop-invariant lane-constants record

Adds a LaneConsts record, formed once per wavefront before the frame loop, that holds each lane's precomputed LDS row, source, twiddle, bit-reversal and image pointers for the 1024-point spectral+harmonic frame kernel. The FFT passes, window load, sum-of-squares and spectral bin reads take these precomputed pointers instead of recomputing index arithmetic from the lane number every frame. A constexpr consistency check verifies that the hoisted offsets equal the original index expressions. The aim is to cut per-frame integer ALU work, at the cost of more live VGPRs across the loop, which may reduce occupancy or cause spills.

```diff
diff --git a/feature-extractor_amd/build.py b/feature-extractor_amd/build.py
--- a/feature-extractor_amd/build.py
+++ b/feature-extractor_amd/build.py
@@ -20,7 +20,7 @@
          ("fx_tracks.hip", "fx_tracks.o", []),
          ("fx_osc_table.hip", "fx_osc_table.o", []),
          ("fx_osc_bundle.hip", "fx_osc_bundle.o", [])] + [(s, s.replace(".cpp", ".o"), []) for s in HOST_SOURCES]
-HEADERS = ["fx_kernels.h", "fx_context.h", "fx_plan.h", "fx_osc_words.h", "fx_wave.hip.h", "fx_lane_exchange.h", "fx_fft.hip.h", "fx_blocks.hip.h", "fx_frame_kernel.hip.h", "fx_pair_kernel.hip.h", "fx_tail_kernels.hip.h", "fx_hop_kernel.hip.h",
+HEADERS = ["fx_kernels.h", "fx_context.h", "fx_plan.h", "fx_osc_words.h", "fx_wave.hip.h", "fx_lane_exchange.h", "fx_lane_consts.hip.h", "fx_fft.hip.h", "fx_blocks.hip.h", "fx_frame_kernel.hip.h", "fx_pair_kernel.hip.h", "fx_tail_kernels.hip.h", "fx_hop_kernel.hip.h",
            os.path.join("..", "..", "include", "fx.h")]
 
 HIPCC_FLAGS = ["--offload-arch=gfx950", "-O3", "-std=c++17", "-fPIC", "-ffp-contract=off",
diff --git a/feature-extractor_amd/csrc/fx_fft.hip.h b/feature-extractor_amd/csrc/fx_fft.hip.h
--- a/feature-extractor_amd/csrc/fx_fft.hip.h
+++ b/feature-extractor_amd/csrc/fx_fft.hip.h
@@ -260,7 +260,7 @@
     wave_fence();
 }
 
-template <int DIGITS> __device__ __forceinline__ int rev4(int x)
+template <int DIGITS> __host__ __device__ __forceinline__ constexpr int rev4(int x)
 {
     unsigned r = __builtin_bitreverse32((unsigned) x) >> (32 - 2 * DIGITS);
     r = ((r & 0x55555555u) << 1) | ((r >> 1) & 0x55555555u);
@@ -288,6 +288,8 @@
 }
 static_assert(Geo<256>::ITEMS_A % Geo<256>::RQ == 0 && Geo<512>::ITEMS_A % Geo<512>::RQ == 0 && Geo<1024>::ITEMS_A % Geo<1024>::RQ == 0
               && Geo<2048>::ITEMS_A % Geo<2048>::RQ == 0 && Geo<4096>::ITEMS_A % Geo<4096>::RQ == 0, "the real image splits only at multiples of RQ");
+
+#include "fx_lane_consts.hip.h"
 
 template <int N, bool INV>
 __device__ __forceinline__ void first_pass_item(const float* x, const f2 (&ta)[9], f2 (&e)[Geo<N>::RA])
@@ -317,8 +319,8 @@
     }
 }
 
-template <int N, bool INV>
-__device__ __forceinline__ void fft_first_pass(const float (&xin)[Geo<N>::P], f2* cbuf, const float (&ftw)[18], int lane)
+template <int N, bool INV, typename LC = LaneConsts<N>>
+__device__ __forceinline__ void fft_first_pass(const float (&xin)[Geo<N>::P], f2* cbuf, const float (&ftw)[18], int lane, const LC* lc = nullptr)
 {
     typedef Geo<N> G;
     constexpr int R = G::RA;
@@ -332,6 +334,7 @@
         if constexpr (RealExchange<N>::USE) {
             static_assert(R == 16 && G::GA == 1, "one 16-element item per lane");
             f2* img = cbuf + RealExchange<N>::row(lane);
+            if constexpr (LC::TRANSFORM) img = lc->row;
 #pragma unroll
             for (int q = 0; q < RealExchange<N>::SLOTS; q++) img[q] = e[RealExchange<N>::stored(q)];
         } else {
@@ -375,22 +378,24 @@
                         twmul<INV>(e[jin + 4], w[3 + 3 * jin]), twmul<INV>(e[jin + 8], w[4 + 3 * jin]), twmul<INV>(e[jin + 12], w[5 + 3 * jin]));
 }
 
-template <int N, bool INV>
-__device__ __forceinline__ void fft_second_pass_regs(const f2* cbuf, const f2* tw, int lane, f2 (&e)[16])
+template <int N, bool INV, typename LC = LaneConsts<N>>
+__device__ __forceinline__ void fft_second_pass_regs(const f2* cbuf, const f2* tw, int lane, f2 (&e)[16], const LC* lc = nullptr)
 {
     typedef Plan<N> PL;
     static_assert(LaneExchange<N>::AVAILABLE && RealExchange<N>::USE && PL::R1 == 16 && PL::L1 == 16 && N / 16 == 64, "one second-pass item per lane");
     const int k = lane % 16;
     const int slot = (int) ((RealExchange<N>::SLOT_OF >> (4 * k)) & 15ull);
-    const unsigned flip = ((RealExchange<N>::TWIN >> k) & 1u) << 31;
+    unsigned flip = ((RealExchange<N>::TWIN >> k) & 1u) << 31;
     const f2* src = cbuf + RealExchange<N>::row((lane / 16) * 16) + slot;
+    const f2* t1 = tw + PL::OFF1 + k;
+    if constexpr (LC::TRANSFORM) { flip = lc->flip; src = lc->src; t1 = lc->tw1; }
 #pragma unroll
     for (int i = 0; i < 16; i++) {
         const f2 v = src[i * RealExchange<N>::SLOTS];
         e[i] = f2{v.x, __uint_as_float(__float_as_uint(v.y) ^ flip)};
     }
     wave_fence();
-    item16_stages<PL::L1, INV>(e, tw + PL::OFF1 + k);
+    item16_stages<PL::L1, INV>(e, t1);
 }
 
 template <bool HALVES> __device__ __forceinline__ void lane_swap(f2& a, f2& b)
@@ -465,8 +470,8 @@
 template <int N> __host__ __device__ constexpr int qpad(int q) { return N == 2048 ? q + 8 * (q >> 6) : q; }
 static_assert(qpad<2048>(1023) < Geo<2048>::CSLOTS && qpad<4096>(2047) < Geo<4096>::CSLOTS, "half image fits the wave buffer");
 
-template <int N, bool INV, int OUT>
-__device__ __forceinline__ float fft_last_pass_consume(f2 (&e)[(N / Plan<N>::R2) / 64][Plan<N>::R2], f2* cbuf, const f2* tw, int lane, float scale, float* regs_out)
+template <int N, bool INV, int OUT, typename LC = LaneConsts<N>>
+__device__ __forceinline__ float fft_last_pass_consume(f2 (&e)[(N / Plan<N>::R2) / 64][Plan<N>::R2], f2* cbuf, const f2* tw, int lane, float scale, float* regs_out, const LC* lc = nullptr)
 {
     typedef Plan<N> PL;
     constexpr int R = PL::R2, L0 = PL::L2, GI = (N / R) / 64, TWOFF = PL::OFF2;
@@ -476,6 +481,7 @@
     for (int g = 0; g < GI; g++) {
         const int k = lane + 64 * g;
         const f2* t1 = tw + TWOFF + k;
+        if constexpr (LC::TRANSFORM) t1 = lc->tw2 + 64 * g;
         if constexpr (R == 16) {
             item16_stages<L0, INV>(e[g], t1);
         } else {
@@ -488,15 +494,17 @@
         for (int i = 0; i < R; i++) {
             const int bin = k + L0 * i;
             if (OUT == OUT_RE_LOW || OUT == OUT_RE_LOW_MAXABS) {
-                if (i < R / 2) fbuf[bimg<N>(lane) + bimg_step<N>(64 * g + L0 * i)] = e[g][i].x;
+                if constexpr (LC::IMAGES) { if (i < R / 2) lc->bin_lane[bimg_step<N>(64 * g + L0 * i)] = e[g][i].x; }
+                else if (i < R / 2) fbuf[bimg<N>(lane) + bimg_step<N>(64 * g + L0 * i)] = e[g][i].x;
                 if (OUT == OUT_RE_LOW_MAXABS && i < R / 4) aux = fmaxf(aux, fmaxf(fabsf(e[g][i].x), fabsf(e[g][i].y)));
             } else if (OUT == OUT_POWER) {
                 if constexpr (Geo<N>::GA == 1) {
                     constexpr int RA = Geo<N>::RA;
                     const int m = g + (L0 / 64) * i;
                     const int j = (RA == 4) ? m : (RA == 8) ? (2 * (m & 3) + (m >> 2)) : (4 * (m & 3) + (m >> 2));
-                    regs_out[j] = __int_as_float(__builtin_amdgcn_ds_bpermute(
-                        rev4<Geo<N>::IDIG>(lane) << 2, __float_as_int(e[g][i].x * e[g][i].x)));
+                    int from = rev4<Geo<N>::IDIG>(lane) << 2;
+                    if constexpr (LC::REV) from = lc->bperm;
+                    regs_out[j] = __int_as_float(__builtin_amdgcn_ds_bpermute(from, __float_as_int(e[g][i].x * e[g][i].x)));
                 } else {
                     fbuf[rimg<N>(lane) + rimg_step<N>(64 * g + L0 * i)] = e[g][i].x * e[g][i].x;
                 }
@@ -527,19 +535,19 @@
     return fft_last_pass_consume<N, INV, OUT>(e, cbuf, tw, lane, scale, regs_out);
 }
 
-template <int N, bool INV, int OUT>
-__device__ __forceinline__ float fft_last_passes_lanes(f2* cbuf, const f2* tw, int lane, float scale, float* regs_out)
+template <int N, bool INV, int OUT, typename LC = LaneConsts<N>>
+__device__ __forceinline__ float fft_last_passes_lanes(f2* cbuf, const f2* tw, int lane, float scale, float* regs_out, const LC* lc = nullptr)
 {
     typedef LaneExchange<N> LX;
     f2 s[16];
-    fft_second_pass_regs<N, INV>(cbuf, tw, lane, s);
+    fft_second_pass_regs<N, INV>(cbuf, tw, lane, s, lc);
     second_exchange_regs<N>(s);
     f2 e[4][4];
 #pragma unroll
     for (int g = 0; g < 4; g++)
 #pragma unroll
         for (int i = 0; i < 4; i++) e[g][i] = s[LX::register_of(g, i)];
-    return fft_last_pass_consume<N, INV, OUT>(e, cbuf, tw, lane, scale, regs_out);
+    return fft_last_pass_consume<N, INV, OUT>(e, cbuf, tw, lane, scale, regs_out, lc);
 }
 
 template <int N, int OUT>
@@ -567,15 +575,17 @@
     const f2* t1;
     float scale;
     int lane;
-    __device__ __forceinline__ void load(const float (&xin)[Geo<N>::P], f2* cbuf, const f2* tw, const float (&ftw)[18], int lane_, float scale_)
+    template <typename LC = LaneConsts<N>>
+    __device__ __forceinline__ void load(const float (&xin)[Geo<N>::P], f2* cbuf, const f2* tw, const float (&ftw)[18], int lane_, float scale_, const LC* lc = nullptr)
     {
-        fft_first_pass<N, true>(xin, cbuf, ftw, lane_);
+        fft_first_pass<N, true>(xin, cbuf, ftw, lane_, lc);
         lane = lane_;
         scale = scale_;
         t1 = tw + PL::OFF2 + lane;
+        if constexpr (LC::TRANSFORM) t1 = lc->tw2;
         if constexpr (lane_exchange_used<N, true, OUT_LAG>()) {
             f2 s[16];
-            fft_second_pass_regs<N, true>(cbuf, tw, lane, s);
+            fft_second_pass_regs<N, true>(cbuf, tw, lane, s, lc);
             second_exchange_regs<N>(s);
 #pragma unroll
             for (int g = 0; g < 4; g++)
@@ -740,19 +750,19 @@
     return aux;
 }
 
-template <int N, bool INV, int OUT, bool CTW = false>
+template <int N, bool INV, int OUT, bool CTW = false, typename LC = LaneConsts<N>>
 __device__ __forceinline__ float fft_from_regs(const float (&xin)[Geo<N>::P], f2* cbuf, const f2* tw, const float (&ftw)[18],
                                                int lane, float scale = 0.0f, float* regs_out = nullptr, const TwRegs<N>* twr = nullptr,
-                                               TwGlobal tg = TwGlobal{nullptr, false, f2{0.0f, 0.0f}})
+                                               TwGlobal tg = TwGlobal{nullptr, false, f2{0.0f, 0.0f}}, const LC* lc = nullptr)
 {
     typedef Plan<N> PL;
     static_assert(!CTW || Geo<N>::SPLIT, "the compact twiddle image belongs to a split transform");
     if constexpr (Geo<N>::SPLIT) {
         return fft_split<N, INV, OUT, CTW>(xin, cbuf, tw, ftw, lane, scale, regs_out, twr, tg);
     } else {
-        fft_first_pass<N, INV>(xin, cbuf, ftw, lane);
+        fft_first_pass<N, INV>(xin, cbuf, ftw, lane, lc);
         if constexpr (lane_exchange_used<N, INV, OUT>()) {
-            return fft_last_passes_lanes<N, INV, OUT>(cbuf, tw, lane, scale, regs_out);
+            return fft_last_passes_lanes<N, INV, OUT>(cbuf, tw, lane, scale, regs_out, lc);
         } else {
             fft_pass<N, PL::R1, PL::L1, PL::OFF1, INV, RealExchange<N>::USE>(cbuf, tw, lane);
             return fft_last_pass_fused<N, INV, OUT>(cbuf, tw, lane, scale, regs_out);
diff --git a/feature-extractor_amd/csrc/fx_frame_kernel.hip.h b/feature-extractor_amd/csrc/fx_frame_kernel.hip.h
--- a/feature-extractor_amd/csrc/fx_frame_kernel.hip.h
+++ b/feature-extractor_amd/csrc/fx_frame_kernel.hip.h
@@ -73,10 +73,10 @@
     }
 }
 
-template <int N, int FMT_A, int FMT_B, bool BLOCKS = false>
+template <int N, int FMT_A, int FMT_B, bool BLOCKS = false, typename LC = LaneConsts<N>>
 __device__ __forceinline__ double load_window(const void* src_a, const void* src_b, float gain_a, float gain_b,
                                               float* rbuf, float* tail_out, int lane, const BlockStream bs = BlockStream{}, const bool a_stream = false,
-                                              const BlockStream bs_a = BlockStream{})
+                                              const BlockStream bs_a = BlockStream{}, const LC* lc = nullptr)
 {
     double ssq = 0.0;
     constexpr int HALF = N / 2, QH = HALF / 256;
@@ -95,14 +95,16 @@
     for (int q = 0; q < QH; q++) {
         const int i = 256 * q + 4 * lane;
         const f4 v = widen_four<FMT_A>(ra[q]) * gain_a;
-        *reinterpret_cast<f4*>(&rbuf[rimg<N>(i)]) = v;
+        if constexpr (LC::IMAGES) *reinterpret_cast<f4*>(lc->load_at + rimg_step<N>(256 * q)) = v;
+        else *reinterpret_cast<f4*>(&rbuf[rimg<N>(i)]) = v;
         if (Geo<N>::SPLIT) ssq += (double) (v.x * v.x) + (double) (v.y * v.y) + (double) (v.z * v.z) + (double) (v.w * v.w);
     }
 #pragma unroll
     for (int q = 0; q < QH; q++) {
         const int i = 256 * q + 4 * lane;
         const f4 v = widen_four<FMT_B>(rb[q]) * gain_b;
-        *reinterpret_cast<f4*>(&rbuf[rimg<N>(HALF + i)]) = v;
+        if constexpr (LC::IMAGES) *reinterpret_cast<f4*>(lc->load_at + rimg_step<N>(HALF + 256 * q)) = v;
+        else *reinterpret_cast<f4*>(&rbuf[rimg<N>(HALF + i)]) = v;
         if (tail_out) *reinterpret_cast<f4*>(tail_out + i) = v;
         if (Geo<N>::SPLIT) ssq += (double) (v.x * v.x) + (double) (v.y * v.y) + (double) (v.z * v.z) + (double) (v.w * v.w);
     }
@@ -250,8 +252,9 @@
 };
 static_assert(FrameLds<4096>::bytes(1, 8, false) <= 160 * 1024 && FrameLds<4096>::bytes(8, 1, true) <= 160 * 1024, "eight 4096-point wavefronts per CU");
 
-template <int N, bool DIRECT = false, bool HOIST = false, bool WIDE = false, bool BLOCKS = false> struct FrameWave {
+template <int N, bool DIRECT = false, bool HOIST = false, bool WIDE = false, bool BLOCKS = false, unsigned LCG = 0u> struct FrameWave {
     typedef Geo<N> G;
+    typedef LaneConsts<N, LCG> LCT;
     static constexpr int M = G::M, P = G::P, U = G::U, HALF = N / 2;
 
     const FrameParams& p;
@@ -266,6 +269,7 @@
     double nyquist, rnyq, frpb;
     float  scale;
     int    c, T, t;
+    const LCT* lc = nullptr;
 
     struct HarmonicSpectrum { float hre[U]; float left2, left1, right1; double sum, max; };
 
@@ -321,7 +325,7 @@
             const void* src_a = sr.a; const void* src_b = sr.b;
             const float gain_a = sr.gain_a, gain_b = sr.gain_b;
             if constexpr (N >= 512) {
-                FX_FORMATS(sr.fmt_a, sr.fmt_b, (ssq = load_window<N, FA, FB, BLOCKS>(src_a, src_b, gain_a, gain_b, rbuf, tail_dst, lane, sr.bs, sr.a_stream, sr.bs_a)));
+                FX_FORMATS(sr.fmt_a, sr.fmt_b, (ssq = load_window<N, FA, FB, BLOCKS>(src_a, src_b, gain_a, gain_b, rbuf, tail_dst, lane, sr.bs, sr.a_stream, sr.bs_a, lc)));
             } else {
                 load_half<N, HALF>(src_a, sr.fmt_a, gain_a, gain_a != 1.0f, rbuf, 0, nullptr, lane);
                 load_half<N, HALF>(src_b, sr.fmt_b, gain_b, gain_b != 1.0f, rbuf, HALF, tail_dst, lane);
@@ -331,13 +335,18 @@
         return ssq;
     }
 
+    __device__ __forceinline__ const float* first_pass_from(int lane, int g) const
+    {
+        if constexpr (LCT::REV) { static_assert(G::GA == 1, "one first-pass item per lane"); return lc->rbase; }
+        else return rbuf + first_pass_rbase<N>(lane, g);
+    }
     __device__ __forceinline__ double sum_squares(int lane, float (&xr)[P]) const
     {
 FX_MARK("rms");
 #pragma unroll
         for (int g = 0; g < G::GA; g++)
 #pragma unroll
-            for (int j = 0; j < G::RA; j++) xr[g * G::RA + j] = (rbuf + first_pass_rbase<N>(lane, g))[first_pass_rstep<N>(j)];
+            for (int j = 0; j < G::RA; j++) xr[g * G::RA + j] = first_pass_from(lane, g)[first_pass_rstep<N>(j)];
         wave_fence();
         double s = 0.0;
 #pragma unroll
@@ -430,6 +439,11 @@
         return pr;
     }
 
+    __device__ __forceinline__ const float* own_bins(int lane) const
+    {
+        if constexpr (LCT::IMAGES) return lc->left2 + LaneOffsets<N>::left_back(2);
+        else return reinterpret_cast<const float*>(cbuf) + bimg<N>(U * lane);
+    }
     __device__ __forceinline__ void spectral(int lane, const float (&xr)[P], double sum_sq) const
     {
         float spec_aux = 0.0f;
@@ -439,8 +453,9 @@
             float xw[P];
 #pragma unroll
             for (int g = 0; g < G::GA; g++) {
-                const float base = (float) rev4<G::IDIG>(lane + 64 * g) * (2.0f / N);
-                const float nbase = 1.0f - base;
+                float base = (float) rev4<G::IDIG>(lane + 64 * g) * (2.0f / N);
+                float nbase = 1.0f - base;
+                if constexpr (LCT::REV) { base = LCT::fresh(lc->base); nbase = 1.0f - base; }
 #pragma unroll
                 for (int j = 0; j < G::RA; j++) {
                     const int r = (G::RA == 4) ? j : (G::RA == 8) ? ((j >> 1) + 4 * (j & 1)) : ((j >> 2) + 4 * (j & 3));
@@ -449,14 +464,14 @@
                     xw[g * G::RA + j] = xr[g * G::RA + j] * gain;
                 }
             }
-            spec_aux = fft_from_regs<N, false, OUT_RE_LOW_MAXABS, WIDE>(xw, cbuf, tw, p.first_tw, lane, 0.0f, nullptr, twr, tw_global());
+            spec_aux = fft_from_regs<N, false, OUT_RE_LOW_MAXABS, WIDE>(xw, cbuf, tw, p.first_tw, lane, 0.0f, nullptr, twr, tw_global(), lc);
         }
         FX_STOP(6, FX_KEEP(spec_aux); return);
 FX_MARK("spec_sums");
         {
             float re[U];
             float maxabs = spec_aux;
-            lds_load_block<U>(reinterpret_cast<const float*>(cbuf) + bimg<N>(U * lane), re);
+            lds_load_block<U>(own_bins(lane), re);
             const float tg = gate_threshold(sum_sq, re);
             double Ts = 0.0, Vs = 0.0, Ws = 0.0, t_after = 0.0;
             double flat_sum = 0.0;
@@ -575,14 +590,21 @@
         float h_max_re = 0.0f;
 FX_MARK("harm1");
         lane = FX_OPQ(2, lane);
-        fft_from_regs<N, false, OUT_RE_LOW, WIDE>(xr, cbuf, tw, p.first_tw, lane, 0.0f, nullptr, twr, tw_global());
+        fft_from_regs<N, false, OUT_RE_LOW, WIDE>(xr, cbuf, tw, p.first_tw, lane, 0.0f, nullptr, twr, tw_global(), lc);
         {
             const int b0 = U * lane;
             const float* relin = reinterpret_cast<const float*>(cbuf);
-            lds_load_block<U>(relin + bimg<N>(b0), hre);
+            lds_load_block<U>(own_bins(lane), hre);
+            if constexpr (LCT::IMAGES) {
+                const float* around = lc->left2;
+                h_left2  = b0 >= 2 ? fabsf(around[0]) : 0.0f;
+                h_left1  = b0 >= 1 ? fabsf(around[1]) : 0.0f;
+                h_right1 = b0 + U < M ? fabsf(around[LaneOffsets<N>::left_back(2) + LaneOffsets<N>::right_step()]) : 0.0f;
+            } else {
             h_left2  = b0 >= 2 ? fabsf(relin[bimg<N>(b0 - 2)]) : 0.0f;
             h_left1  = b0 >= 1 ? fabsf(relin[bimg<N>(b0 - 1)]) : 0.0f;
             h_right1 = b0 + U < M ? fabsf(relin[bimg<N>(b0 + U)]) : 0.0f;
+            }
 #pragma unroll
             for (int j = 0; j < U; j++) {
                 const double v = (double) hre[j];
@@ -613,7 +635,7 @@
         float x[P];
 #pragma unroll
         for (int i = 0; i < P; i += 4) {
-            const f4 v = *reinterpret_cast<const f4*>(&rbuf[rimg<N>(P * lane + i)]);
+            const f4 v = *reinterpret_cast<const f4*>(LCT::IMAGES ? lc->warm + LaneOffsets<N>::warmup_back() + i : &rbuf[rimg<N>(P * lane + i)]);
             x[i] = v.x; x[i + 1] = v.y; x[i + 2] = v.z; x[i + 3] = v.w;
         }
         float yin = 0.0f;
@@ -623,7 +645,7 @@
             for (int q = 0; q < KW / 4; q++) {
                 const int n0 = first - KW + 4 * q;
                 if (n0 >= 0) {
-                    const f4 v = *reinterpret_cast<const f4*>(&rbuf[rimg<N>(n0)]);
+                    const f4 v = *reinterpret_cast<const f4*>(LCT::IMAGES ? lc->warm + 4 * q : &rbuf[rimg<N>(n0)]);
                     const float w[4] = {v.x, v.y, v.z, v.w};
                     float aw[4];
                     scaled_pairs<4>(a, w, aw);
@@ -664,8 +686,9 @@
             }
         }
         lane = FX_OPQ(3, lane);
-        const float w0 = bartlett_gain<N>(P * lane);
-        const float wstep = lane < 32 ? (2.0f / N) : -(2.0f / N);
+        float w0 = bartlett_gain<N>(P * lane);
+        float wstep = lane < 32 ? (2.0f / N) : -(2.0f / N);
+        if constexpr (LCT::IMAGES) { w0 = LCT::fresh(lc->w0); wstep = lc->wstep; }
 #pragma unroll
         for (int i = 0; i < P; i += 4) {
             f4 v;
@@ -673,7 +696,7 @@
             v.y = y[i + 1] * __builtin_fmaf(wstep, (float) (i + 1), w0);
             v.z = y[i + 2] * __builtin_fmaf(wstep, (float) (i + 2), w0);
             v.w = y[i + 3] * __builtin_fmaf(wstep, (float) (i + 3), w0);
-            *reinterpret_cast<f4*>(&rbuf[rimg<N>(P * lane + i)]) = v;
+            *reinterpret_cast<f4*>(LCT::IMAGES ? lc->warm + LaneOffsets<N>::warmup_back() + i : &rbuf[rimg<N>(P * lane + i)]) = v;
         }
         wave_fence();
     }
@@ -722,10 +745,10 @@
 #pragma unroll
         for (int g = 0; g < G::GA; g++)
 #pragma unroll
-            for (int j = 0; j < G::RA; j++) xf[g * G::RA + j] = (rbuf + first_pass_rbase<N>(lane, g))[first_pass_rstep<N>(j)];
+            for (int j = 0; j < G::RA; j++) xf[g * G::RA + j] = first_pass_from(lane, g)[first_pass_rstep<N>(j)];
         wave_fence();
         float xp[P];
-        fft_from_regs<N, false, OUT_POWER, WIDE>(xf, cbuf, tw, p.first_tw, lane, 0.0f, xp, twr, tw_global());
+        fft_from_regs<N, false, OUT_POWER, WIDE>(xf, cbuf, tw, p.first_tw, lane, 0.0f, xp, twr, tw_global(), lc);
         FX_STOP(3, for (int j = 0; j < P; j++) FX_KEEP(xp[j]); return 1.0);
 FX_MARK("power");
         lane = FX_OPQ(7, lane);
@@ -744,7 +767,7 @@
         float lag;
         if constexpr (N == 1024) {
             LazyLag<N> lz;
-            lz.load(xf, cbuf, tw, p.first_tw, lane, scale);
+            lz.load(xf, cbuf, tw, p.first_tw, lane, scale, lc);
             vreg[0] = lz.head(0);
             vreg[1] = lz.head(1);
             FX_STOP(4, FX_KEEP(vreg[0]); FX_KEEP(vreg[1]); return 1.0);
@@ -866,6 +889,11 @@
     }
 };
 
+template <int N, bool SPEC, bool HARM, bool DIRECT, bool BLOCKS> constexpr unsigned lane_consts_groups()
+{
+    return (N == 1024 && SPEC && HARM && !DIRECT && !BLOCKS) ? LANE_CONSTS_GROUPS : 0u;
+}
+
 template <int N, bool SPEC, bool HARM, bool DIRECT, bool BLOCKS = false>
 __device__ __forceinline__ void frame_kernel_body(const FrameParams& p_arg)
 {
@@ -939,6 +967,9 @@
 
     TwRegs<N> twr;
     if constexpr (TwRegs<N>::USE) twr.load(tw, lane0);
+    constexpr unsigned LCG = lane_consts_groups<N, SPEC, HARM, DIRECT, BLOCKS>();
+    LaneConsts<N, LCG> lcs;
+    if constexpr (LCG != 0u) lcs.form(lane0, cbuf, tw);
 
     const double nyquist = p.nyquist;
     const double rnyq = 1.0 / nyquist;
@@ -954,10 +985,10 @@
     };
     for (int t = live ? (CLAIM ? next_frame(0) : t_begin + slot) : t_end; t < t_end; t = next_frame(t)) {
         constexpr bool HOIST = SPEC && !HARM && N == 1024;
-        const int lane = FX_OPQ(15, lane0);
+        const int lane = LaneConsts<N, LCG>::TOP ? lane0 : FX_OPQ(15, lane0);
         FramePart* fpl = p.part + ((size_t) c * T + t);
         if (lane == 0) fpl->flags = 0;
-        const FrameWave<N, DIRECT, HOIST, WIDE, BLOCKS> w{p, tw, &twr, prev, turn, cbuf, rbuf, fpl, nyquist, rnyq, frpb, scale, c, T, t};
+        const FrameWave<N, DIRECT, HOIST, WIDE, BLOCKS, LCG> w{p, tw, &twr, prev, turn, cbuf, rbuf, fpl, nyquist, rnyq, frpb, scale, c, T, t, &lcs};
 
         const double ssq_lane = w.load_frame(lane);
         float xr[P];
@@ -979,7 +1010,7 @@
         }
         FX_STOP(6, continue); FX_STOP(7, continue); FX_STOP(8, continue); FX_STOP(9, continue); FX_STOP(10, continue);
         if constexpr (HARM) {
-            typename FrameWave<N, DIRECT, HOIST, WIDE, BLOCKS>::HarmonicSpectrum hs;
+            typename FrameWave<N, DIRECT, HOIST, WIDE, BLOCKS, LCG>::HarmonicSpectrum hs;
             if constexpr (G::SPLIT) w.template load_raw<true>(lane, xr);
             w.harmonic_spectrum(lane, xr, hs);
             FX_STOP(11, FX_KEEP(hs.sum); FX_KEEP(hs.max); FX_KEEP(hs.left2); FX_KEEP(hs.left1); FX_KEEP(hs.right1); for (int j = 0; j < G::U; j++) FX_KEEP(hs.hre[j]); continue);
diff --git a/feature-extractor_amd/csrc/fx_lane_consts.hip.h b/feature-extractor_amd/csrc/fx_lane_consts.hip.h
--- /dev/null
+++ b/feature-extractor_amd/csrc/fx_lane_consts.hip.h
@@ -0,0 +1,114 @@
+enum { LCG_TRANSFORM = 1, LCG_REV = 2, LCG_IMAGES = 4, LCG_TOP = 8, LCG_ALL = 15 };
+
+template <int N> struct LaneOffsets {
+    typedef Geo<N> G;
+    typedef RealExchange<N> RX;
+    typedef Plan<N> PL;
+    __host__ __device__ static constexpr int row(int lane) { return RX::row(lane); }
+    __host__ __device__ static constexpr int src(int lane) { return RX::row((lane / 16) * 16) + (int) ((RX::SLOT_OF >> (4 * (lane % 16))) & 15ull); }
+    __host__ __device__ static constexpr unsigned flip(int lane) { return ((RX::TWIN >> (lane % 16)) & 1u) << 31; }
+    __host__ __device__ static constexpr int tw1(int lane) { return PL::OFF1 + lane % PL::L1; }
+    __host__ __device__ static constexpr int tw2(int lane) { return PL::OFF2 + lane; }
+    __host__ __device__ static constexpr int rev(int lane) { return rev4<G::IDIG>(lane); }
+    __host__ __device__ static constexpr int rbase(int lane) { return rimg<N>(rev(lane)); }
+    __host__ __device__ static constexpr int load_at(int lane) { return rimg<N>(4 * lane); }
+    __host__ __device__ static constexpr int own(int lane) { return rimg<N>(G::P * lane); }
+    __host__ __device__ static constexpr int bins(int lane) { return bimg<N>(G::U * lane); }
+    __host__ __device__ static constexpr int bin_lane(int lane) { return bimg<N>(lane); }
+
+    __host__ __device__ static constexpr int rev_by_digits(int x)
+    {
+        int r = 0;
+        for (int d = 0; d < G::IDIG; d++) { r = 4 * r + (x & 3); x >>= 2; }
+        return r;
+    }
+    __host__ __device__ static constexpr bool consistent()
+    {
+        for (int lane = 0; lane < 64; lane++) {
+            const int k = lane % 16;
+            int slot = -1;
+            for (int q = 0; q < RX::SLOTS; q++)
+                if (RX::stored(q) == k || (((RX::TWIN >> k) & 1u) && RX::stored(q) == (k == 12 ? 4 : 16 - k))) slot = q;
+            if (slot < 0 || src(lane) != ((lane / 16) * 16) * RX::SLOTS + slot) return false;
+            if (row(lane) != lane * RX::SLOTS || row(lane) + RX::SLOTS > cpad(N) + 2) return false;
+            const bool twin = k == 3 || k == 7 || k == 11 || k == 12 || k == 15;
+            if (flip(lane) != (twin ? 0x80000000u : 0u)) return false;
+            if (tw1(lane) != k || tw2(lane) != 15 * 16 + lane || tw2(lane) + 64 * 3 + 2 * PL::L2 >= N) return false;
+            if (rev(lane) != rev_by_digits(lane) || rev(lane) >= G::ITEMS_A) return false;
+            for (int j = 0; j < G::RA; j++) {
+                const int r = (j >> 2) + 4 * (j & 3);
+                if (rbase(lane) + first_pass_rstep<N>(j) != rimg<N>(rev(lane) + G::ITEMS_A * r)) return false;
+            }
+            for (int q = 0; q < N / 512; q++)
+                if (load_at(lane) + rimg_step<N>(256 * q) != rimg<N>(256 * q + 4 * lane)
+                    || load_at(lane) + rimg_step<N>(N / 2 + 256 * q) != rimg<N>(N / 2 + 256 * q + 4 * lane)) return false;
+            for (int i = 0; i < G::P; i++)
+                if (own(lane) + i != rimg<N>(G::P * lane + i)) return false;
+            if (lane > 0)
+                for (int i = 0; i < 16; i++)
+                    if (own(lane) - warmup_back() + i != rimg<N>(G::P * lane - 16 + i)) return false;
+            for (int j = 0; j < G::U; j++)
+                if (bins(lane) + j != bimg<N>(G::U * lane + j)) return false;
+            if (lane > 0 && (bins(lane) - left_back(2) != bimg<N>(G::U * lane - 2) || bins(lane) - left_back(1) != bimg<N>(G::U * lane - 1))) return false;
+            if (lane < 63 && bins(lane) + right_step() != bimg<N>(G::U * lane + G::U)) return false;
+            for (int m = 0; m < G::U; m++)
+                if (bin_lane(lane) + bimg_step<N>(64 * m) != bimg<N>(lane + 64 * m)) return false;
+        }
+        return true;
+    }
+    __host__ __device__ static constexpr int warmup_back() { return 16 + 4 * (16 / G::RQ); }
+    __host__ __device__ static constexpr int left_back(int n) { return n + (G::BQ ? 4 : 0); }
+    __host__ __device__ static constexpr int right_step() { return G::U + (G::BQ ? 4 : 0); }
+};
+static_assert(LaneOffsets<1024>::consistent(), "LaneConsts: a member plus its section's constant is the index the section forms from the lane number");
+
+#define FX_LC_TEXT_(x) #x
+#define FX_LC_TEXT(x) FX_LC_TEXT_(x)
+constexpr unsigned LANE_CONSTS_SHIPPED = LCG_TRANSFORM | LCG_REV | LCG_IMAGES;
+constexpr unsigned LANE_CONSTS_GROUPS = lds_exchange_kinds(FX_LC_TEXT(FX_EXP_LANE_CONSTS), LANE_CONSTS_SHIPPED);
+static_assert(LANE_CONSTS_GROUPS <= (unsigned) LCG_ALL, "FX_EXP_LANE_CONSTS: a mask of the four groups of members");
+
+template <int N, unsigned GROUPS = 0u> struct LaneConsts {
+    static constexpr bool TRANSFORM = (GROUPS & LCG_TRANSFORM) != 0, REV = (GROUPS & LCG_REV) != 0, IMAGES = (GROUPS & LCG_IMAGES) != 0, TOP = (GROUPS & LCG_TOP) != 0;
+    static_assert(GROUPS == 0u || N == 1024, "the record belongs to the 1024-point frame kernel");
+    typedef LaneOffsets<N> O;
+    f2*        row;
+    const f2*  src;
+    unsigned   flip;
+    const f2*  tw1;
+    const f2*  tw2;
+    const float* rbase;
+    int        bperm;
+    float      base;
+    float*     load_at;
+    float*     warm;
+    float*     left2;
+    float*     bin_lane;
+    float      w0, wstep;
+    static __device__ __forceinline__ float fresh(float v) { asm volatile("" : "+v"(v)); return v; }
+
+    __device__ __forceinline__ void form(int lane, f2* cbuf, const f2* tw)
+    {
+        float* rbuf = reinterpret_cast<float*>(cbuf);
+        if constexpr (TRANSFORM) {
+            row = cbuf + O::row(lane);
+            src = cbuf + O::src(lane);
+            flip = O::flip(lane);
+            tw1 = tw + O::tw1(lane);
+            tw2 = tw + O::tw2(lane);
+        }
+        if constexpr (REV) {
+            rbase = rbuf + O::rbase(lane);
+            bperm = O::rev(lane) << 2;
+            base = (float) O::rev(lane) * (2.0f / N);
+        }
+        if constexpr (IMAGES) {
+            load_at = rbuf + O::load_at(lane);
+            warm = rbuf + O::own(lane) - O::warmup_back();
+            left2 = rbuf + O::bins(lane) - O::left_back(2);
+            bin_lane = rbuf + O::bin_lane(lane);
+            w0 = bartlett_gain<N>(Geo<N>::P * lane);
+            wstep = lane < 32 ? (2.0f / N) : -(2.0f / N);
+        }
+    }
+};
```

After: 201.2 million, median of 6. 1.02x the previous value.
